# zhang-tao-whu/DVIS_Plus

Measured on AMD Instinct MI355X. Metric: frames/sec DVIS++ R50 offline, 720p T=30 synthetic, higher is better.
Workload: dtype f32 (storage, accumulation, results; the segmenter's dense layers - R50 convolutions from 128 channels on, pixel-decoder projections and FPN output convolution, the deformable encoder's projections and FFN, the decoder's key / value projections - multiply each fp32 operand as two f16 terms on the f1

## Files before the change

dvis_plus_amd/csrc/conv1x1_x3.hip:

```cpp
#include "dvis_common.h"
#include "x3_common.h"

DVIS_EXPORT int64_t dvis_conv_x3_image_bytes(int64_t N, int C, int H, int W);

namespace {

constexpr unsigned kOOB = 0x80000000u;

struct CxArgs {
  const float *x, *bias, *res;
  const void *wp;
  float *y;
  int N, C, K, relu, npass;
  int stride, W_in, OW, H_in;
  int taps;
  long long HW, HW_in, pixels;
  long long tiles;
  float xscale, inv;
  int *flag;
  int tag;
  const float *x2;
  int C2, stride2, W2_in;
  long long HW2_in;
  void *img;
  int XG;
  float oscale;
  int OH;
  const void *ximg;
  int XG_in;
};

__device__ __forceinline__ bool cx_item(const CxArgs &a, long long w, long long *tile, int *pass) {
  const int xcd = blockIdx.x & 7, i = blockIdx.x >> 3, per = gridDim.x >> 3;
  const long long m = i + (long long)per * w;
  const long long u = m / a.npass;
  *pass = (int)(m - u * a.npass);
  *tile = xcd + 8 * u;
  return *tile < a.tiles;
}

struct CxGeom {
  unsigned base;
  int iy, ix;
  int row0;
};
__device__ __forceinline__ CxGeom cx_geom(const CxArgs &a, long long p) {
  CxGeom gm = {kOOB, 0, 0, 0};
  if (p >= a.pixels) return gm;
  const long long n = p / a.HW;
  const int pix = (int)(p - n * a.HW);
  const int oy = pix / a.OW, ox = pix - oy * a.OW, pad = a.taps == 9 ? 1 : 0;
  gm.base = (unsigned)(n * a.C * a.HW_in * 4);
  gm.iy = oy * a.stride - pad, gm.ix = ox * a.stride - pad;
  gm.row0 = (int)(n * a.H_in);
  return gm;
}
__device__ __forceinline__ unsigned cx_tap_offset(const CxArgs &a, const CxGeom &gm, int tap) {
  const int dy = a.taps == 9 ? tap / 3 : 0, dx = a.taps == 9 ? tap - 3 * dy : 0;
  const int iy = gm.iy + dy, ix = gm.ix + dx;
  const bool ok = gm.base != kOOB && iy >= 0 && iy < a.H_in && ix >= 0 && ix < a.W_in;
  return ok ? gm.base + (unsigned)((iy * a.W_in + ix) * 4) : kOOB;
}

__device__ __forceinline__ unsigned cx_tap_offset_img(const CxArgs &a, const CxGeom &gm, int tap, int g) {
  const int dy = a.taps == 9 ? tap / 3 : 0, dx = a.taps == 9 ? tap - 3 * dy : 0;
  const int iy = gm.iy + dy, ix = gm.ix + dx;
  const bool ok = gm.base != kOOB && iy >= 0 && iy < a.H_in && ix >= 0 && ix < a.W_in;
  return ok ? (unsigned)(((gm.row0 + iy) * a.XG_in + (ix >> 5)) * ((a.C / 64) * 8192) + g * 512 + (ix & 31) * 16) : kOOB;
}

__device__ __forceinline__ unsigned cx_geom2(const CxArgs &a, long long p) {
  if (a.C2 == 0 || p >= a.pixels) return kOOB;
  const long long n = p / a.HW;
  const int pix = (int)(p - n * a.HW);
  const int oy = pix / a.OW, ox = pix - oy * a.OW;
  return (unsigned)(n * a.C2 * a.HW2_in * 4) + (unsigned)((oy * a.stride2 * a.W2_in + ox * a.stride2) * 4);
}

template <int NB, int NW, int IK, bool IMGIN = false, bool IMGOUT = false>
__global__ __launch_bounds__(NW * 64) void conv1x1_x3_kernel(const CxArgs a) {
  constexpr int kTile = NW * 32, PW = 2 * IK * NB / NW, STAGES = IK == 4 ? 2 : 3, IPC = 4 / IK;
  static_assert(2 * IK * NB % NW == 0, "the item's pieces must divide among the waves");
  extern __shared__ __attribute__((aligned(1024))) char lds[];
  const int wave = threadIdx.x >> 6, lane = threadIdx.x & 63, j = lane & 31, g = lane >> 5;
  const int NCC = a.C / 64, NC1 = a.taps * NCC, NC = NC1 + a.C2 / 64, NI = IPC * NC;
  long long wcount = 0;
  {
    long long t;
    int q;
    while (cx_item(a, wcount, &t, &q)) ++wcount;
  }
  if (wcount == 0) return;
  const __amdgpu_buffer_rsrc_t rx = dvis_make_rsrc_uniform(a.x, (unsigned)((long long)a.N * a.C * a.HW_in * 4));
  const __amdgpu_buffer_rsrc_t ry = dvis_make_rsrc_uniform(a.y, (unsigned)((long long)a.N * a.K * a.HW * 4));
  const __amdgpu_buffer_rsrc_t rr = dvis_make_rsrc_uniform(a.res ? a.res : a.y, (unsigned)((long long)a.N * a.K * a.HW * 4));
  const unsigned chan = (unsigned)(a.HW_in * 4);
  const __amdgpu_buffer_rsrc_t rx2 = dvis_make_rsrc_uniform(a.C2 ? a.x2 : a.x, a.C2 ? (unsigned)((long long)a.N * a.C2 * a.HW2_in * 4) : 0u);
  const unsigned chan2 = (unsigned)(a.HW2_in * 4);

  typedef Ring<PW, IMGIN ? 8 : 32, NW, STAGES> RingT;
  RingT ring;
  long long iw = 0;
  int ic = 0, ipass;
  {
    long long t;
    cx_item(a, 0, &t, &ipass);
  }
  auto next_offset = [&]() -> size_t {
    const size_t o = ((size_t)ipass * NI + ic) * RingT::kItemBytes;
    if (++ic == NI) {
      ic = 0;
      long long t;
      if (!cx_item(a, ++iw, &t, &ipass)) ipass = 0;
    }
    return o;
  };
  ring.init(a.wp, lds, 1, (int)(wcount * NI), wave, lane);
#pragma unroll
  for (int i = 0; i < RingT::kAhead; ++i)
    if (ring.total > i) ring.issue_at(next_offset());

  float raw[32];
  auto load_raw = [&](unsigned pixoff, int cc, bool second = false) {
    const __amdgpu_buffer_rsrc_t r = second ? rx2 : rx;
    const unsigned ch = second ? chan2 : chan;
    const unsigned vo = pixoff + (unsigned)(8 * g) * ch;
    const unsigned so = (unsigned)(64 * cc) * ch;
#pragma unroll
    for (int s = 0; s < 4; ++s)
#pragma unroll
      for (int e = 0; e < 8; ++e)
        raw[8 * s + e] = __builtin_bit_cast(float, __builtin_amdgcn_raw_buffer_load_b32(r, vo, so + (unsigned)(16 * s + e) * ch, 0));
  };
  const __amdgpu_buffer_rsrc_t rxi = dvis_make_rsrc_uniform(IMGIN ? a.ximg : (const void *)a.x,
                                                            IMGIN ? (unsigned)((long long)a.N * a.H_in * a.XG_in * (a.C / 64) * 8192) : 0u);
  h8 nh[4], nl[4];
  auto load_img = [&](unsigned off, int cc) {
#pragma unroll
    for (int s = 0; s < 4; ++s) {
      nh[s] = __builtin_bit_cast(h8, __builtin_amdgcn_raw_buffer_load_b128(rxi, off, (unsigned)(8192 * cc + 2048 * s), 0));
      nl[s] = __builtin_bit_cast(h8, __builtin_amdgcn_raw_buffer_load_b128(rxi, off, (unsigned)(8192 * cc + 2048 * s + 1024), 0));
    }
  };
  long long tile;
  int pass;
  cx_item(a, 0, &tile, &pass);
  CxGeom gm = cx_geom(a, tile * kTile + wave * 32 + j);
  unsigned gm2 = cx_geom2(a, tile * kTile + wave * 32 + j);
  if constexpr (IMGIN)
    load_img(cx_tap_offset_img(a, gm, 0, g), 0);
  else
    load_raw(cx_tap_offset(a, gm, 0), 0);
  for (long long w = 0; w < wcount; ++w) {
    const long long p = tile * kTile + wave * 32 + j;
    long long ntile = tile;
    int npass_ = pass;
    const bool more = cx_item(a, w + 1, &ntile, &npass_);
    const CxGeom ngm = more ? cx_geom(a, ntile * kTile + wave * 32 + j) : CxGeom{kOOB, 0, 0, 0};
    const unsigned ngm2 = more ? cx_geom2(a, ntile * kTile + wave * 32 + j) : kOOB;
    int tap = 0, cc = 0;
    f16v acc[NB];
#pragma unroll
    for (int nb = 0; nb < NB; ++nb)
#pragma unroll
      for (int i = 0; i < 16; ++i) acc[nb][i] = 0.f;
    const long long n = p / a.HW;
    const unsigned obase = p < a.pixels ? (unsigned)((n * a.K * a.HW + (p - n * a.HW)) * 4) : kOOB;
    const unsigned ochan = (unsigned)(a.HW * 4);
    const int co0 = pass * 32 * NB;
    for (int kc = 0; kc < NC; ++kc) {
      h8 xh[4], xl[4];
      if constexpr (IMGIN) {
#pragma unroll
        for (int s = 0; s < 4; ++s) {
          asm volatile("" : "+v"(nh[s]), "+v"(nl[s]));
          xh[s] = nh[s], xl[s] = nl[s];
        }
        if (++cc == NCC) cc = 0, ++tap;
        const bool first = kc + 1 < NC1;
        load_img(first ? cx_tap_offset_img(a, gm, tap, g) : cx_tap_offset_img(a, ngm, 0, g), first ? cc : 0);
      } else {
#pragma unroll
        for (int i = 0; i < 32; ++i) asm volatile("" : "+v"(raw[i]));
#pragma unroll
        for (int s = 0; s < 4; ++s) {
          const f4 lo4 = {raw[8 * s], raw[8 * s + 1], raw[8 * s + 2], raw[8 * s + 3]};
          const f4 hi4 = {raw[8 * s + 4], raw[8 * s + 5], raw[8 * s + 6], raw[8 * s + 7]};
          split8(lo4, hi4, a.xscale, xh[s], xl[s]);
        }
        if (++cc == NCC) cc = 0, ++tap;
        const bool first = kc + 1 < NC1, sec = !first && kc + 1 < NC;
        const unsigned po = first ? cx_tap_offset(a, gm, tap) : (sec ? gm2 : cx_tap_offset(a, ngm, 0));
        load_raw(po, first ? cc : (sec ? kc + 1 - NC1 : 0), sec);
      }
#pragma unroll
      for (int part = 0; part < IPC; ++part) {
        const char *stage = ring.wait(false);
        ring.begin(ring.more() ? next_offset() : 0);
        mma_item<IK, NB, PW>(stage, lane, acc, xh + IK * part, xl + IK * part, [&](int i) { ring.piece(i); });
      }
    }
    float chk = 0.f;
    if constexpr (NB == 2 || IMGOUT) {
      if (a.img != nullptr) {
        const unsigned gs = (unsigned)(a.K / 64) * 8192u;
        const __amdgpu_buffer_rsrc_t ri = dvis_make_rsrc_uniform(a.img, (unsigned)((long long)a.N * a.OH * a.XG * gs));
        const __amdgpu_buffer_rsrc_t rb = dvis_make_rsrc_uniform(a.bias ? (const void *)a.bias : (const void *)a.img, a.bias ? (unsigned)a.K * 4u : 0u);
        unsigned ibase = kOOB;
        if (p < a.pixels) {
          const int pix = (int)(p - n * a.HW), oy = pix / a.OW, ox = pix - oy * a.OW;
          ibase = (unsigned)(((n * a.OH + oy) * a.XG + (ox >> 5)) * gs + (co0 / 64) * 8192 + g * 512 + (ox & 31) * 16);
        }
#pragma unroll
        for (int nb = 0; nb < NB; ++nb) {
          float v[16];
#pragma unroll
          for (int q = 0; q < 4; ++q) {
            const f4 b = __builtin_bit_cast(f4, __builtin_amdgcn_raw_buffer_load_b128(rb, (unsigned)(co0 + 32 * nb + 8 * q + 4 * g) * 4u, 0, 0));
#pragma unroll
            for (int i = 0; i < 4; ++i) {
              const float t = acc[nb][4 * q + i] * a.inv + b[i];
              chk = __builtin_fmaf(t, 0.f, chk);
              v[4 * q + i] = a.relu ? x3_relu(t) : t;
            }
          }
          h8 hi[2], lo[2];
#pragma unroll
          for (int u = 0; u < 2; ++u) {
            const f4 p0 = {v[8 * u], v[8 * u + 1], v[8 * u + 2], v[8 * u + 3]}, p1 = {v[8 * u + 4], v[8 * u + 5], v[8 * u + 6], v[8 * u + 7]};
            split8(p0, p1, a.oscale, hi[u], lo[u]);
          }
          const h8 ls = lo[0] + lo[1];
          chk = __builtin_fmaf((float)((ls[0] + ls[1]) + (ls[2] + ls[3]) + (ls[4] + ls[5]) + (ls[6] + ls[7])), 0.f, chk);
          store_fragments4(ri, ibase, hi[0], 4096 * nb, lo[0], 4096 * nb + 1024, hi[1], 4096 * nb + 2048, lo[1], 4096 * nb + 3072);
        }
        if (a.flag != nullptr && chk != chk && p < a.pixels) atomicCAS(a.flag, 0, a.tag);
        tile = ntile, pass = npass_, gm = ngm, gm2 = ngm2;
        continue;
      }
    }
#pragma unroll
    for (int nb = 0; nb < NB; ++nb) {
      float rv[16];
#pragma unroll
      for (int r = 0; r < 16; ++r)
        rv[r] = a.res ? __builtin_bit_cast(float, __builtin_amdgcn_raw_buffer_load_b32(
                                                      rr, obase + (unsigned)(co0 + 32 * nb + 8 * (r >> 2) + 4 * g + (r & 3)) * ochan, 0, 0))
                      : 0.f;
#pragma unroll
      for (int q = 0; q < 4; ++q) {
        const int co = co0 + 32 * nb + 8 * q + 4 * g;
        f4 b = {0.f, 0.f, 0.f, 0.f};
        if (a.bias) b = *(const f4 *)(a.bias + co);
#pragma unroll
        for (int i = 0; i < 4; ++i) {
          const unsigned o = obase + (unsigned)(co + i) * ochan;
          float v = acc[nb][4 * q + i] * a.inv + b[i] + rv[4 * q + i];
          chk = __builtin_fmaf(v, 0.f, chk);
          if (a.relu) v = x3_relu(v);
          __builtin_amdgcn_raw_buffer_store_b32(__builtin_bit_cast(unsigned, v), ry, o, 0, 0);
        }
      }
    }
    if (a.flag != nullptr && chk != chk && p < a.pixels) atomicCAS(a.flag, 0, a.tag);
    tile = ntile, pass = npass_, gm = ngm, gm2 = ngm2;
  }
}

__global__ __launch_bounds__(256) void upsample_add_image_kernel(const float *__restrict__ lateral, const float *__restrict__ top,
                                                                 void *__restrict__ img, int N, int C, int H, int W, int h, int w,
                                                                 const float *__restrict__ lat_scale, const float *__restrict__ lat_shift,
                                                                 float oscale) {
  const int NCC = C / 64, XG = (W + 31) / 32;
  const int cc = blockIdx.x, xg = blockIdx.y;
  const int x = threadIdx.x & 31, g = (threadIdx.x >> 5) & 1, S = threadIdx.x >> 6;
  const int px = 32 * xg + x;
  const float sy = (float)h / (float)H, sx = (float)w / (float)W;
  const int pxc = px < W ? px : W - 1;
  float fx = sx * ((float)pxc + 0.5f) - 0.5f;
  fx = fx < 0.f ? 0.f : fx;
  const int x0 = min((int)fx, w - 1), x1 = x0 + (x0 < w - 1 ? 1 : 0);
  const float lx1 = fx - (float)x0, lx0 = 1.f - lx1;
  const __amdgpu_buffer_rsrc_t ri = dvis_make_rsrc_uniform(img, (unsigned)((long long)N * H * XG * NCC * 8192));
  const unsigned rows = (unsigned)N * (unsigned)H;
  for (unsigned row = blockIdx.z * 16u; row < blockIdx.z * 16u + 16u && row < rows; ++row) {
    const unsigned n = row / (unsigned)H;
    const int y = (int)(row - n * (unsigned)H);
    float fy = sy * ((float)y + 0.5f) - 0.5f;
    fy = fy < 0.f ? 0.f : fy;
    const int y0 = min((int)fy, h - 1), y1 = y0 + (y0 < h - 1 ? 1 : 0);
    const float ly1 = fy - (float)y0, ly0 = 1.f - ly1;
    float v[8];
#pragma unroll
    for (int e = 0; e < 8; ++e) {
      const int c = 64 * cc + 32 * (S >> 1) + 16 * (S & 1) + 8 * (e >> 2) + 4 * g + (e & 3);
      const unsigned pl = n * (unsigned)C + (unsigned)c;
      const float *t0 = top + ((size_t)pl * h + y0) * (size_t)w, *t1 = top + ((size_t)pl * h + y1) * (size_t)w;
      float lat = lateral[((size_t)pl * H + y) * (size_t)W + pxc];
      if (lat_scale) lat = lat * lat_scale[pl] + lat_shift[pl];
      v[e] = lat + (ly0 * (lx0 * t0[x0] + lx1 * t0[x1]) + ly1 * (lx0 * t1[x0] + lx1 * t1[x1]));
    }
    const f4 p0 = {v[0], v[1], v[2], v[3]}, p1 = {v[4], v[5], v[6], v[7]};
    h8 hi, lo;
    split8(p0, p1, oscale, hi, lo);
    const unsigned G = row * (unsigned)XG + (unsigned)xg;
    const unsigned off = (G * (unsigned)NCC + (unsigned)cc) * 8192u + (unsigned)(S * 2048 + g * 512 + x * 16);
    store_fragments2(ri, off, hi, 0, lo, 1024);
  }
}

}

DVIS_EXPORT int dvis_upsample_add_image(const float *lateral, const float *lat_scale, const float *lat_shift, const float *top, void *image,
                                        int N, int C, int H, int W, int h, int w, int oexp, void *stream) {
  DVIS_REQUIRE(lateral && top && image, "dvis_upsample_add_image: null pointer");
  DVIS_REQUIRE((lat_scale == nullptr) == (lat_shift == nullptr), "dvis_upsample_add_image: scale and shift together");
  DVIS_REQUIRE(N > 0 && C > 0 && C % 64 == 0 && H > 0 && W > 0 && h > 0 && w > 0, "dvis_upsample_add_image: bad sizes");
  DVIS_REQUIRE((uintptr_t)image % 16 == 0 && dvis_conv_x3_image_bytes(N, C, H, W) < ((int64_t)1 << 31), "dvis_upsample_add_image: a 16-byte "
               "aligned image below 2 GiB");
  const int per = 16 * 65535 / H;
  DVIS_REQUIRE(per >= 1 && (W + 31) / 32 <= 65535, "dvis_upsample_add_image: map too large (%d x %d)", H, W);
  for (int i = 0; i < N; i += per) {
    const int n = N - i < per ? N - i : per;
    hipLaunchKernelGGL(upsample_add_image_kernel, dim3(C / 64, (W + 31) / 32, (n * H + 15) / 16), dim3(256), 0, (hipStream_t)stream,
                       lateral + (size_t)i * C * H * W, top + (size_t)i * C * h * w,
                       (char *)image + (size_t)i * H * ((W + 31) / 32) * (C / 64) * 8192, n, C, H, W, h, w,
                       lat_scale ? lat_scale + (size_t)i * C : nullptr, lat_shift ? lat_shift + (size_t)i * C : nullptr, ldexpf(1.f, oexp));
  }
  return dvis_check_launch("dvis_upsample_add_image");
}

DVIS_EXPORT int dvis_conv1x1_x3_supported(int C, int K, int64_t N, int64_t HW_in, int64_t HW_out) {
  if (C < 64 || C % 64 != 0 || C > 4096) return 0;
  if (!(K == 64 || K == 128 || (K > 0 && K % 256 == 0 && K <= 8192))) return 0;
  if (N <= 0 || HW_out <= 0 || HW_in < HW_out) return 0;
  if (N * C * HW_in * 4 >= ((int64_t)1 << 31) || N * K * HW_out * 4 >= ((int64_t)1 << 31)) return 0;
  return 1;
}

DVIS_EXPORT int64_t dvis_conv1x1_x3_packed_bytes(int C, int K) {
  if (!dvis_conv1x1_x3_supported(C, K, 1, 1, 1)) return -1;
  return (int64_t)(C / 16) * (K / 32) * 2 * kPiece;
}

DVIS_EXPORT int dvis_conv1x1_x3_pack(const float *w, int K, int C, int wexp, void *packed, void *stream) {
  DVIS_REQUIRE(w && packed, "dvis_conv1x1_x3_pack: null operand");
  DVIS_REQUIRE(dvis_conv1x1_x3_supported(C, K, 1, 1, 1), "dvis_conv1x1_x3_pack: (C, K) = (%d, %d) is not served", C, K);
  DVIS_REQUIRE(wexp >= -60 && wexp <= 60, "dvis_conv1x1_x3_pack: wexp = %d", wexp);
  const int NB = K == 64 ? 2 : K == 128 ? 4 : 8;
  const int64_t fragments = (int64_t)(C / 16) * (K / 32) * 64;
  hipLaunchKernelGGL(x3_pack_kernel, dim3((unsigned)((fragments + 255) / 256)), dim3(256), 0, (hipStream_t)stream, w, (int64_t)C, K, C,
                     NB, 0, ldexpf(1.f, wexp), (_Float16 *)packed, fragments);
  return dvis_check_launch("dvis_conv1x1_x3_pack");
}

static int cx_launch(const float *x, const void *packed, const float *bias, const float *res, float *y, int N, int C, int K, int H, int W,
                     int stride, int taps, int xexp, int wexp, int relu, void *stream, const float *x2 = nullptr, int C2 = 0, int H2 = 0,
                     int W2 = 0, int stride2 = 1, void *image = nullptr, int oexp = 0, const void *ximg = nullptr);

DVIS_EXPORT int dvis_conv1x1_x3_dual(const float *x, const float *x2, const void *packed, const float *bias, const float *res, float *y,
                                     int N, int C, int C2, int K, int H, int W, int H2, int W2, int stride2, int xexp, int wexp, int relu,
                                     void *stream) {
  DVIS_REQUIRE(x2 != nullptr && C2 >= 64 && C2 % 64 == 0 && C2 <= 4096, "dvis_conv1x1_x3_dual: C2 %% 64 == 0 (got %d)", C2);
  DVIS_REQUIRE((stride2 == 1 || stride2 == 2) && (H2 + stride2 - 1) / stride2 == H && (W2 + stride2 - 1) / stride2 == W,
               "dvis_conv1x1_x3_dual: x2 (%d x %d, stride %d) must down-sample onto x's %d x %d map", H2, W2, stride2, H, W);
  DVIS_REQUIRE((long long)N * C2 * H2 * W2 * 4 < ((long long)1 << 31) && (uintptr_t)x2 % 16 == 0, "dvis_conv1x1_x3_dual: x2 below 2 GiB, 16-byte aligned");
  return cx_launch(x, packed, bias, res, y, N, C, K, H, W, 1, 1, xexp, wexp, relu, stream, x2, C2, H2, W2, stride2);
}

DVIS_EXPORT int dvis_conv1x1_x3(const float *x, const void *packed, const float *bias, const float *res, float *y, int N, int C, int K,
                                int H, int W, int stride, int xexp, int wexp, int relu, void *stream) {
  return cx_launch(x, packed, bias, res, y, N, C, K, H, W, stride, 1, xexp, wexp, relu, stream);
}

DVIS_EXPORT int dvis_conv1x1_x3_image(const float *x, const void *packed, const float *bias, void *image, int N, int C, int H, int W, int xexp,
                                      int wexp, int oexp, int relu, void *stream) {
  DVIS_REQUIRE(image != nullptr && (uintptr_t)image % 16 == 0, "dvis_conv1x1_x3_image: null / unaligned image");
  DVIS_REQUIRE((long long)N * H * ((W + 31) / 32) * 8192 < ((long long)1 << 31), "dvis_conv1x1_x3_image: the image must stay below 2 GiB");
  return cx_launch(x, packed, bias, nullptr, nullptr, N, C, 64, H, W, 1, 1, xexp, wexp, relu, stream, nullptr, 0, 0, 0, 1, image, oexp);
}

DVIS_EXPORT int64_t dvis_conv_x3_image_bytes(int64_t N, int C, int H, int W) {
  if (N < 0 || C <= 0 || C % 64 != 0 || H <= 0 || W <= 0) return -1;
  return N * H * ((W + 31) / 32) * (int64_t)(C / 64) * 8192;
}

DVIS_EXPORT int dvis_conv_x3_pack_image(const float *w, int K, int C, int taps, int wexp, void *packed, void *stream) {
  DVIS_REQUIRE(w && packed, "dvis_conv_x3_pack_image: null operand");
  DVIS_REQUIRE(taps == 1 || taps == 9, "dvis_conv_x3_pack_image: taps = %d", taps);
  DVIS_REQUIRE(dvis_conv1x1_x3_supported(C, K, 1, 1, 1) && K >= 128, "dvis_conv_x3_pack_image: (C, K) = (%d, %d) is not served", C, K);
  DVIS_REQUIRE(wexp >= -60 && wexp <= 60, "dvis_conv_x3_pack_image: wexp = %d", wexp);
  const int NB = K == 128 ? 4 : 8;
  const int64_t fragments = (int64_t)(taps * C / 16) * (K / 32) * 64;
  hipLaunchKernelGGL(x3_pack_kernel, dim3((unsigned)((fragments + 255) / 256)), dim3(256), 0, (hipStream_t)stream, w, (int64_t)taps * C, K,
                     taps * C, NB, 1, ldexpf(1.f, wexp), (_Float16 *)packed, fragments, taps);
  return dvis_check_launch("dvis_conv_x3_pack_image");
}

DVIS_EXPORT int dvis_conv_x3_image(const void *ximg, const float *x, const void *packed, const float *bias, const float *res, float *y,
                                   void *image, int N, int C, int K, int H, int W, int stride, int taps, int xexp, int wexp, int oexp, int relu,
                                   void *stream) {
  DVIS_REQUIRE(ximg != nullptr || image != nullptr, "dvis_conv_x3_image: neither side is an operand image (use dvis_conv1x1_x3 / dvis_conv3x3_x3)");
  DVIS_REQUIRE((ximg != nullptr) != (x != nullptr), "dvis_conv_x3_image: exactly one of ximg and x");
  DVIS_REQUIRE((image != nullptr) != (y != nullptr), "dvis_conv_x3_image: exactly one of image and y");
  DVIS_REQUIRE(K == 128 || K % 256 == 0, "dvis_conv_x3_image: K = %d (128 or a multiple of 256)", K);
  DVIS_REQUIRE(taps == 1 || taps == 9, "dvis_conv_x3_image: taps = %d", taps);
  DVIS_REQUIRE(image == nullptr || res == nullptr, "dvis_conv_x3_image: an image output takes no residual");
  DVIS_REQUIRE(((uintptr_t)ximg | (uintptr_t)image) % 16 == 0, "dvis_conv_x3_image: images must be 16-byte aligned");
  const int OH = (H + stride - 1) / stride, OW = (W + stride - 1) / stride;
  DVIS_REQUIRE(dvis_conv_x3_image_bytes(N, C, H, W) < ((int64_t)1 << 31) && dvis_conv_x3_image_bytes(N, K, OH, OW) < ((int64_t)1 << 31),
               "dvis_conv_x3_image: images must stay below 2 GiB");
  return cx_launch(x, packed, bias, res, y, N, C, K, H, W, stride, taps, xexp, wexp, relu, stream, nullptr, 0, 0, 0, 1, image, oexp, ximg);
}

DVIS_EXPORT int64_t dvis_conv3x3_x3_packed_bytes(int C, int K) {
  const int64_t b = dvis_conv1x1_x3_packed_bytes(C, K);
  return b < 0 ? b : 9 * b;
}

DVIS_EXPORT int dvis_conv3x3_x3_pack(const float *w, int K, int C, int wexp, void *packed, void *stream) {
  DVIS_REQUIRE(w && packed, "dvis_conv3x3_x3_pack: null operand");
  DVIS_REQUIRE(dvis_conv1x1_x3_supported(C, K, 1, 1, 1), "dvis_conv3x3_x3_pack: (C, K) = (%d, %d) is not served", C, K);
  DVIS_REQUIRE(wexp >= -60 && wexp <= 60, "dvis_conv3x3_x3_pack: wexp = %d", wexp);
  const int NB = K == 64 ? 2 : K == 128 ? 4 : 8;
  const int64_t fragments = (int64_t)(9 * C / 16) * (K / 32) * 64;
  hipLaunchKernelGGL(x3_pack_kernel, dim3((unsigned)((fragments + 255) / 256)), dim3(256), 0, (hipStream_t)stream, w, (int64_t)9 * C, K, 9 * C,
                     NB, 0, ldexpf(1.f, wexp), (_Float16 *)packed, fragments, 9);
  return dvis_check_launch("dvis_conv3x3_x3_pack");
}

DVIS_EXPORT int dvis_conv3x3_x3(const float *x, const void *packed, const float *bias, const float *res, float *y, int N, int C, int K,
                                int H, int W, int stride, int xexp, int wexp, int relu, void *stream) {
  return cx_launch(x, packed, bias, res, y, N, C, K, H, W, stride, 9, xexp, wexp, relu, stream);
}

static int cx_launch(const float *x, const void *packed, const float *bias, const float *res, float *y, int N, int C, int K, int H, int W,
                     int stride, int taps, int xexp, int wexp, int relu, void *stream, const float *x2, int C2, int H2, int W2, int stride2,
                     void *image, int oexp, const void *ximg) {
  DVIS_REQUIRE((x || ximg) && packed && (y || image), "dvis_conv1x1_x3: null operand");
  DVIS_REQUIRE(stride == 1 || stride == 2, "dvis_conv1x1_x3: stride %d", stride);
  const int OH = (H + stride - 1) / stride, OW = (W + stride - 1) / stride;
  DVIS_REQUIRE(dvis_conv1x1_x3_supported(C, K, N, (int64_t)H * W, (int64_t)OH * OW), "dvis_conv1x1_x3: shape (N %d, C %d, K %d, %d x %d, "
               "stride %d) is not served (C %% 64 == 0, K = 64 / 128 or K %% 256 == 0, tensors below 2 GiB)", N, C, K, H, W, stride);
  DVIS_REQUIRE((uintptr_t)x % 16 == 0 && (uintptr_t)y % 16 == 0 && (uintptr_t)packed % 16 == 0 && (bias == nullptr || (uintptr_t)bias % 16 == 0),
               "dvis_conv1x1_x3: operands must be 16-byte aligned");
  CxArgs a = {};
  a.x = x, a.bias = bias, a.res = res, a.wp = packed, a.y = y, a.N = N, a.C = C, a.K = K, a.relu = relu;
  a.stride = stride, a.W_in = W, a.H_in = H, a.taps = taps, a.OW = OW, a.HW = (long long)OH * OW, a.HW_in = (long long)H * W;
  a.pixels = a.HW * N;
  a.xscale = ldexpf(1.f, xexp), a.inv = ldexpf(1.f, -(xexp + wexp));
  const X3Guard gd = dvis_x3_guard();
  a.flag = gd.flag, a.tag = gd.tag;
  a.x2 = x2, a.C2 = x2 ? C2 : 0, a.stride2 = stride2, a.W2_in = W2, a.HW2_in = (long long)H2 * W2;
  a.img = image, a.XG = (OW + 31) / 32, a.oscale = ldexpf(1.f, oexp), a.OH = OH;
  a.ximg = ximg, a.XG_in = (W + 31) / 32;
  const int grid = dvis_x3_persistent_cus();
  hipStream_t st = (hipStream_t)stream;
  static const int nw = getenv("DVIS_X3_CONV_WAVES") ? atoi(getenv("DVIS_X3_CONV_WAVES")) : 8;
  a.npass = K <= 128 ? 1 : K / 256;
#define DVIS_CX_LAUNCH(NBV, NWV, IKV)                                                                              \
  {                                                                                                                \
    static DvisLdsOptIn opted;                                                                                     \
    typedef Ring<2 * IKV * NBV / NWV, 32, NWV, (IKV == 4 ? 2 : 3)> R;                                              \
    a.tiles = (a.pixels + 32 * NWV - 1) / (32 * NWV);                                                              \
    const size_t lds = (IKV == 4 ? 2 : 3) * R::kItemBytes;                                                         \
    const int rc = dvis_lds_opt_in((const void *)conv1x1_x3_kernel<NBV, NWV, IKV>, lds, &opted, "dvis_conv1x1_x3"); \
    if (rc != DVIS_OK) return rc;                                                                                  \
    hipLaunchKernelGGL((conv1x1_x3_kernel<NBV, NWV, IKV>), dim3(grid), dim3(NWV * 64), lds, st, a);                \
  }
#define DVIS_CX_LAUNCH_IMG(NBV, IKV, INV, OUTV)                                                                                    \
  {                                                                                                                                \
    static DvisLdsOptIn opted;                                                                                                     \
    typedef Ring<2 * IKV * NBV / 8, 8, 8, (IKV == 4 ? 2 : 3)> R;                                                                   \
    a.tiles = (a.pixels + 255) / 256;                                                                                              \
    const size_t lds = (IKV == 4 ? 2 : 3) * R::kItemBytes;                                                                         \
    const int rc = dvis_lds_opt_in((const void *)conv1x1_x3_kernel<NBV, 8, IKV, INV, OUTV>, lds, &opted, "dvis_conv_x3_image");    \
    if (rc != DVIS_OK) return rc;                                                                                                  \
    hipLaunchKernelGGL((conv1x1_x3_kernel<NBV, 8, IKV, INV, OUTV>), dim3(grid), dim3(512), lds, st, a);                            \
    return dvis_check_launch("dvis_conv_x3_image");                                                                                \
  }
  if (ximg != nullptr || (image != nullptr && K != 64)) {
    DVIS_REQUIRE(x2 == nullptr, "dvis_conv_x3_image: no second source");
    if (K == 128) {
      if (ximg && image) DVIS_CX_LAUNCH_IMG(4, 2, true, true)
      if (ximg) DVIS_CX_LAUNCH_IMG(4, 2, true, false)
      DVIS_CX_LAUNCH_IMG(4, 2, false, true)
    }
    if (ximg && image) DVIS_CX_LAUNCH_IMG(8, 4, true, true)
    if (ximg) DVIS_CX_LAUNCH_IMG(8, 4, true, false)
    DVIS_CX_LAUNCH_IMG(8, 4, false, true)
  }
#undef DVIS_CX_LAUNCH_IMG
  static const int ik = getenv("DVIS_X3_CONV_ITEM") ? atoi(getenv("DVIS_X3_CONV_ITEM")) : 4;
  if (K == 64) {
    if (nw == 8) DVIS_CX_LAUNCH(2, 8, 2) else DVIS_CX_LAUNCH(2, 4, 2)
  } else if (K == 128) {
    if (nw == 8) DVIS_CX_LAUNCH(4, 8, 2) else DVIS_CX_LAUNCH(4, 4, 2)
  } else if (ik == 4) {
    DVIS_CX_LAUNCH(8, 8, 4)
  } else {
    if (nw == 8) DVIS_CX_LAUNCH(8, 8, 2) else DVIS_CX_LAUNCH(8, 4, 2)
  }
#undef DVIS_CX_LAUNCH
  return dvis_check_launch("dvis_conv1x1_x3");
}
```

dvis_plus_amd/csrc/fused_elementwise.hip:

```cpp
#include <math.h>

#include "dvis_common.h"

namespace {

template <int V>
__global__ __launch_bounds__(256) void add_layernorm_kernel(const float *__restrict__ x, const float *__restrict__ res,
                                                            int64_t res_row_stride, const float *__restrict__ gamma,
                                                            const float *__restrict__ beta, float *__restrict__ out,
                                                            size_t rows, int C, float eps,
                                                            const float *__restrict__ pos, size_t pos_rows,
                                                            float *__restrict__ out_pos) {
  const int lane = threadIdx.x & 63;
  const size_t row = (size_t)blockIdx.x * 4 + (threadIdx.x >> 6);
  if (row >= rows) return;
  const float4 *xr = reinterpret_cast<const float4 *>(x + row * C);
  const float4 *rr = res ? reinterpret_cast<const float4 *>(res + row * res_row_stride) : nullptr;
  float4 v[V];
  float sum = 0.f;
#pragma unroll
  for (int i = 0; i < V; ++i) {
    const int c4 = lane + 64 * i;
    if (c4 * 4 < C) {
      v[i] = xr[c4];
// ... 481 lines not shown

DVIS_EXPORT int dvis_add_layernorm(const float *x, const float *res, int64_t res_row_stride, const float *gamma,
                                   const float *beta, float *out, int64_t rows, int C, float eps, void *stream) {
  return add_layernorm_launch(x, res, res_row_stride, gamma, beta, out, rows, C, eps, nullptr, 0, nullptr, stream);
}

DVIS_EXPORT int dvis_add_layernorm_pos(const float *x, const float *res, int64_t res_row_stride, const float *gamma,
                                       const float *beta, float *out, const float *pos, int64_t pos_rows, float *out_pos,
                                       int64_t rows, int C, float eps, void *stream) {
  DVIS_REQUIRE(pos && out_pos, "add_layernorm_pos: null pos / out_pos");
  return add_layernorm_launch(x, res, res_row_stride, gamma, beta, out, rows, C, eps, pos, pos_rows, out_pos, stream);
}

static int upsample_add_launch(const float *lateral, const float *top, float *out, int64_t planes, int H, int W, int h,
                               int w, const float *lat_scale, const float *lat_shift, void *stream) {
  DVIS_REQUIRE(planes >= 0 && H > 0 && W > 0 && h > 0 && w > 0, "upsample_add: bad sizes");
  if (planes == 0) return DVIS_OK;
  DVIS_REQUIRE(lateral && top && out, "upsample_add: null pointer");
  DVIS_REQUIRE((lat_scale == nullptr) == (lat_shift == nullptr), "upsample_add: scale and shift come together");
  DVIS_REQUIRE(planes < (1ll << 31), "upsample_add: too many planes");
  if (W % 4 != 0 || (((uintptr_t)lateral | (uintptr_t)out) & 15) != 0) {
    const long long tot = (long long)planes * H * W;
    long long nb = (tot + 255) / 256;
    if (nb > 256 * 32) nb = 256 * 32;
    hipLaunchKernelGGL(upsample_add_scalar_kernel, dim3((unsigned)nb), dim3(256), 0, (hipStream_t)stream, lateral, top, out, tot, H, W,
                       h, w, lat_scale, lat_shift);
    return dvis_check_launch("upsample_add_scalar_kernel");
  }
  const size_t total = (size_t)planes * H * (W / 4);
  size_t blocks = (total + 255) / 256;
  if (blocks > 256 * 32) blocks = 256 * 32;
  DVIS_REQUIRE(total < (1ull << 32), "upsample_add: more than 2^32 output quads");
  const bool x2 = H == 2 * h && W == 2 * w && (w & 1) == 0 && ((uintptr_t)top & 7) == 0;
  if (x2)
    hipLaunchKernelGGL(upsample_add_kernel<true>, dim3((unsigned)blocks), dim3(256), 0, (hipStream_t)stream, lateral, top,
                       out, (int)planes, H, W, h, w, lat_scale, lat_shift);
  else
    hipLaunchKernelGGL(upsample_add_kernel<false>, dim3((unsigned)blocks), dim3(256), 0, (hipStream_t)stream, lateral, top,
                       out, (int)planes, H, W, h, w, lat_scale, lat_shift);
  return dvis_check_launch("upsample_add_kernel");
}

DVIS_EXPORT int dvis_dwconv3x3_tokens(const float *x, float *out, int64_t batch_stride, int B, int h, int w, int C, const float *weight,
                                      const float *bias, int gelu, void *stream) {
  DVIS_REQUIRE(x && out && weight, "dwconv3x3_tokens: null pointer");
  DVIS_REQUIRE(B >= 0 && h > 0 && w > 0 && C > 0 && C % 4 == 0 && batch_stride % 4 == 0 && batch_stride >= (int64_t)h * w * C,
               "dwconv3x3_tokens: C %% 4 == 0 and a batch stride that is a multiple of 4 floats >= h * w * C are required");
  DVIS_REQUIRE(((uintptr_t)x | (uintptr_t)out | (uintptr_t)(bias ? bias : weight)) % 16 == 0, "dwconv3x3_tokens: 16-byte alignment");
  DVIS_REQUIRE(x != out, "dwconv3x3_tokens: in place is not possible (neighbouring tokens are read)");
  if (B == 0) return DVIS_OK;
  const int64_t strips = (int64_t)h * ((w + 3) / 4);
  DVIS_REQUIRE(strips * B < ((int64_t)1 << 32), "dwconv3x3_tokens: too many tokens");
  hipLaunchKernelGGL(dwconv3x3_tokens_kernel, dim3((unsigned)((strips * B + 3) / 4), (C / 4 + 63) / 64), dim3(256), 0, (hipStream_t)stream, x,
                     out, batch_stride, B, h, w, C, weight, bias, gelu);
  return dvis_check_launch("dwconv3x3_tokens_kernel");
}

DVIS_EXPORT int dvis_adapter_res2(const float *g, const float *c1, const float *x1, const float *scale, const float *shift, float *out,
                                  int B, int C, int h8, int w8, void *stream) {
  DVIS_REQUIRE(g && c1 && scale && shift && out, "adapter_res2: null pointer");
  DVIS_REQUIRE(((uintptr_t)g | (uintptr_t)c1 | (uintptr_t)out) % 16 == 0, "adapter_res2: g / c1 / out must be 16-byte aligned");
  DVIS_REQUIRE(B >= 0 && C > 0 && C % 64 == 0 && h8 > 0 && w8 > 0 && h8 % 2 == 0 && w8 % 2 == 0,
               "adapter_res2: C %% 64 == 0 and an even stride-8 grid are required (C %d, grid %d x %d)", C, h8, w8);
  DVIS_REQUIRE((int64_t)B * h8 <= 65535 && C / 64 <= 65535, "adapter_res2: grid too large (B * rows %lld)", (long long)B * h8);
  if (B == 0) return DVIS_OK;
  hipLaunchKernelGGL(adapter_res2_kernel, dim3((w8 + 31) / 32, C / 64, B * h8), dim3(256), 0, (hipStream_t)stream, g, c1, x1, scale, shift,
                     out, C, h8, w8);
  return dvis_check_launch("adapter_res2_kernel");
}

DVIS_EXPORT int dvis_upsample_add(const float *lateral, const float *top, float *out, int64_t planes, int H, int W, int h,
                                  int w, void *stream) {
  return upsample_add_launch(lateral, top, out, planes, H, W, h, w, nullptr, nullptr, stream);
}

DVIS_EXPORT int dvis_upsample_add_affine(const float *lateral, const float *lat_scale, const float *lat_shift,
                                         const float *top, float *out, int64_t planes, int H, int W, int h, int w,
                                         void *stream) {
  DVIS_REQUIRE(lat_scale && lat_shift, "upsample_add_affine: null scale / shift");
  return upsample_add_launch(lateral, top, out, planes, H, W, h, w, lat_scale, lat_shift, stream);
}

DVIS_EXPORT int dvis_bias_relu_maxpool(const float *x, const float *bias, float *out, int64_t planes, int C, int H, int W,
                                       void *stream) {
  DVIS_REQUIRE(planes >= 0 && C > 0 && H > 0 && W > 0, "bias_relu_maxpool: bad sizes");
  if (planes == 0) return DVIS_OK;
  DVIS_REQUIRE(x && out, "bias_relu_maxpool: null pointer");
  DVIS_REQUIRE(H % 2 == 0 && W % 8 == 0 && (((uintptr_t)x | (uintptr_t)out) & 15) == 0,
               "bias_relu_maxpool: needs even H, W %% 8 == 0 and 16-byte aligned x / out (H=%d W=%d)", H, W);
  const size_t total = (size_t)planes * (H / 2) * (W / 8);
  DVIS_REQUIRE(planes < (1ll << 31) && total < (1ull << 32), "bias_relu_maxpool: too many planes / outputs");
  size_t blocks = (total + 255) / 256;
  if (blocks > 256 * 32) blocks = 256 * 32;
  hipLaunchKernelGGL(bias_relu_maxpool_kernel, dim3((unsigned)blocks), dim3(256), 0, (hipStream_t)stream, x, bias, out,
                     (int)planes, C, H, W);
  return dvis_check_launch("bias_relu_maxpool_kernel");
}

namespace {

__global__ __launch_bounds__(1024) void group_norm_affine_kernel(const float *__restrict__ x, const float *__restrict__ gamma,
                                                                 const float *__restrict__ beta, float *__restrict__ scale,
                                                                 float *__restrict__ shift, int C, int G, long long HW,
                                                                 float eps, int vec) {
  __shared__ double s_sum[16], s_sq[16];
  const int Cg = C / G;
  const int n = blockIdx.x / G, g = blockIdx.x - n * G;
  const long long count = (long long)Cg * HW, count4 = count / 4;
  const float4 *xp = reinterpret_cast<const float4 *>(x + ((size_t)n * C + (size_t)g * Cg) * HW);
  double sum = 0.0, sq = 0.0;
  if (vec) {
    for (long long i = threadIdx.x; i < count4; i += 1024) {
      const float4 v = xp[i];
      sum += ((double)v.x + (double)v.y) + ((double)v.z + (double)v.w);
      sq += ((double)v.x * v.x + (double)v.y * v.y) + ((double)v.z * v.z + (double)v.w * v.w);
    }
  } else {
    const float *xs = reinterpret_cast<const float *>(xp);
    for (long long i = threadIdx.x; i < count; i += 1024) {
      const double v = (double)xs[i];
      sum += v;
      sq += v * v;
    }
  }
#pragma unroll
  for (int o = 32; o > 0; o >>= 1) {
    sum += __shfl_down(sum, o);
    sq += __shfl_down(sq, o);
  }
  const int wv = threadIdx.x >> 6;
  if ((threadIdx.x & 63) == 0) {
    s_sum[wv] = sum;
    s_sq[wv] = sq;
  }
  __syncthreads();
  if (threadIdx.x < Cg) {
    double ts = 0.0, tq = 0.0;
#pragma unroll
    for (int i = 0; i < 16; ++i) {
      ts += s_sum[i];
      tq += s_sq[i];
    }
    const double mean = ts / (double)count;
    double var = tq / (double)count - mean * mean;
    var = var < 0.0 ? 0.0 : var;
    const float rstd = (float)(1.0 / sqrt(var + (double)eps));
    const int c = g * Cg + threadIdx.x;
    const float a = rstd * (gamma ? gamma[c] : 1.f);
    scale[(size_t)n * C + c] = a;
    shift[(size_t)n * C + c] = (beta ? beta[c] : 0.f) - (float)mean * a;
  }
}

__global__ __launch_bounds__(256) void scale_shift_act_kernel(float *__restrict__ x, const float *__restrict__ scale,
                                                              const float *__restrict__ shift, int HW4, int chunks, int relu) {
  const unsigned plane = blockIdx.x / chunks;
  const int chunk = blockIdx.x - plane * chunks;
  const float a = scale[plane], b = shift[plane];
  float4 *xp = reinterpret_cast<float4 *>(x) + (size_t)plane * HW4;
  for (int i = chunk * 256 + threadIdx.x; i < HW4; i += chunks * 256) {
    float4 v = xp[i];
    v.x = v.x * a + b; v.y = v.y * a + b; v.z = v.z * a + b; v.w = v.w * a + b;
    if (relu) {
      v.x = fmaxf(v.x, 0.f); v.y = fmaxf(v.y, 0.f); v.z = fmaxf(v.z, 0.f); v.w = fmaxf(v.w, 0.f);
    }
    xp[i] = v;
  }
}

__global__ __launch_bounds__(256) void scale_shift_act_scalar_kernel(float *__restrict__ x, const float *__restrict__ scale,
                                                                     const float *__restrict__ shift, long long HW, long long total,
                                                                     int relu) {
  for (long long i = (long long)blockIdx.x * 256 + threadIdx.x; i < total; i += (long long)gridDim.x * 256) {
    const long long plane = i / HW;
    const float v = x[i] * scale[plane] + shift[plane];
    x[i] = relu ? fmaxf(v, 0.f) : v;
  }
}

}

DVIS_EXPORT int dvis_group_norm_affine(const float *x, const float *gamma, const float *beta, float *scale, float *shift,
                                       int64_t N, int C, int G, int64_t HW, float eps, void *stream) {
  DVIS_REQUIRE(N >= 0 && C > 0 && G > 0 && HW > 0 && C % G == 0, "group_norm_affine: bad sizes (C=%d G=%d)", C, G);
  if (N == 0) return DVIS_OK;
  DVIS_REQUIRE(x && scale && shift, "group_norm_affine: null pointer");
  DVIS_REQUIRE(C / G <= 1024, "group_norm_affine: at most 1024 channels per group");
  const int vec = ((int64_t)(C / G) * HW) % 4 == 0 && ((uintptr_t)x & 15) == 0;
  DVIS_REQUIRE(N * G < (1ll << 31), "group_norm_affine: too many groups");
  hipLaunchKernelGGL(group_norm_affine_kernel, dim3((unsigned)(N * G)), dim3(1024), 0, (hipStream_t)stream, x, gamma, beta,
                     scale, shift, C, G, (long long)HW, eps, vec);
  return dvis_check_launch("group_norm_affine_kernel");
}

DVIS_EXPORT int dvis_scale_shift_act(float *x, const float *scale, const float *shift, int64_t planes, int64_t HW, int relu,
                                     void *stream) {
  DVIS_REQUIRE(planes >= 0 && HW > 0, "scale_shift_act: bad sizes");
  if (planes == 0) return DVIS_OK;
  DVIS_REQUIRE(x && scale && shift, "scale_shift_act: null pointer");
  if (HW % 4 != 0 || ((uintptr_t)x & 15) != 0) {
    const long long total = (long long)planes * HW;
    const long long blocks = (total + 255) / 256;
    hipLaunchKernelGGL(scale_shift_act_scalar_kernel, dim3((unsigned)(blocks > 65535 * 16 ? 65535 * 16 : blocks)), dim3(256), 0,
                       (hipStream_t)stream, x, scale, shift, (long long)HW, total, relu);
    return dvis_check_launch("scale_shift_act_scalar_kernel");
  }
  const int HW4 = (int)(HW / 4);
  int chunks = (HW4 + 1023) / 1024;
  if (chunks < 1) chunks = 1;
  DVIS_REQUIRE(planes * chunks < (1ll << 31), "scale_shift_act: too many planes");
  hipLaunchKernelGGL(scale_shift_act_kernel, dim3((unsigned)(planes * chunks)), dim3(256), 0, (hipStream_t)stream, x, scale,
                     shift, HW4, chunks, relu);
  return dvis_check_launch("scale_shift_act_kernel");
}
```

dvis_plus_amd/functions.py:

```python
import collections
import ctypes
import math
import os
import threading

import torch
from torch.autograd import Function
from torch.autograd.function import once_differentiable

from . import cpu_ops, derived, native
from .cpu_ops import ms_deform_attn_core_pytorch


def _torch_path(op, x, why):
    if os.environ.get("DVIS_STRICT", "1") != "0" and x.is_cuda and not torch.is_grad_enabled():
        raise RuntimeError(f"DVIS_STRICT: {op} would run its torch formulation on a GPU tensor ({why}; shape "
                           f"{tuple(x.shape)}, dtype {x.dtype}, contiguous {x.is_contiguous()})")


class no_autocast:

    def __enter__(self):
        import contextlib
        self._stack = contextlib.ExitStack()
# ... 524 lines not shown
        dq, dk, dv = attention_backward(q, k, v, grad_out, ctx.nheads)
        need = ctx.needs_input_grad
        return dq if need[0] else None, dk if need[1] else None, dv if need[2] else None, None, None


def vps_argmax(mask_logits_kthw, scores, first_resize_size, img_size, out_hw):
    K, T, h, w = mask_logits_kthw.shape
    m = mask_logits_kthw
    if not m.is_cuda or m.dtype != torch.float32 or m.stride(3) != 1 or m.stride(2) != w:
        raise RuntimeError("vps_argmax: logits must be a float32 GPU (K, T, h, w) view with contiguous (h, w) maps")
    scores = scores.to(torch.float32).contiguous()
    oh, ow = int(out_hw[0]), int(out_hw[1])
    ids = torch.empty((T, oh, ow), dtype=torch.int32, device=m.device)
    conf = torch.empty((T, oh, ow), dtype=torch.uint8, device=m.device)
    areas = torch.empty((3, K), dtype=torch.int32, device=m.device)
    with torch.cuda.device(m.device):
        rc = native.lib().dvis_vps_argmax(
            ctypes.c_void_p(m.data_ptr()), m.stride(0), m.stride(1), native.dev_ptr(scores, "scores"), K, T, h, w,
            int(first_resize_size[0]), int(first_resize_size[1]), int(img_size[0]), int(img_size[1]), oh, ow,
            native.dev_ptr(ids, "ids"), native.dev_ptr(conf, "conf"), native.dev_ptr(areas, "areas"),
            native.stream_ptr(m.device))
    native.check(rc, "dvis_vps_argmax")
    return ids, conf.bool(), areas


def resize2_gt0(mask_logits_kthw, first_resize_size, img_size, out_hw):
    K, T, h, w = mask_logits_kthw.shape
    m = mask_logits_kthw
    if not m.is_cuda or m.dtype != torch.float32 or m.stride(3) != 1 or m.stride(2) != w:
        raise RuntimeError("resize2_gt0: logits must be a float32 GPU (K, T, h, w) view with contiguous (h, w) maps")
    oh, ow = int(out_hw[0]), int(out_hw[1])
    out = torch.empty((K, T, oh, ow), dtype=torch.uint8, device=m.device)
    with torch.cuda.device(m.device):
        rc = native.lib().dvis_resize2_gt0(
            ctypes.c_void_p(m.data_ptr()), m.stride(0), m.stride(1), K, T, h, w, int(first_resize_size[0]),
            int(first_resize_size[1]), int(img_size[0]), int(img_size[1]), oh, ow, native.dev_ptr(out, "out"),
            native.stream_ptr(m.device))
    native.check(rc, "dvis_resize2_gt0")
    return out.view(torch.bool)


def resize2(mask_logits_kthw, first_resize_size, img_size, out_hw, sigmoid=False):
    K, T, h, w = mask_logits_kthw.shape
    m = mask_logits_kthw
    if not m.is_cuda or m.dtype != torch.float32 or m.stride(3) != 1 or m.stride(2) != w:
        raise RuntimeError("resize2: logits must be a float32 GPU (K, T, h, w) view with contiguous (h, w) maps")
    oh, ow = int(out_hw[0]), int(out_hw[1])
    out = torch.empty((K, T, oh, ow), dtype=torch.float32, device=m.device)
    with torch.cuda.device(m.device):
        rc = native.lib().dvis_resize2(
            ctypes.c_void_p(m.data_ptr()), m.stride(0), m.stride(1), K, T, h, w, int(first_resize_size[0]),
            int(first_resize_size[1]), int(img_size[0]), int(img_size[1]), oh, ow, 1 if sigmoid else 0,
            native.dev_ptr(out, "out"), native.stream_ptr(m.device))
    native.check(rc, "dvis_resize2")
    return out


def vss_argmax(mask_logits_qthw, mask_cls, first_resize_size, img_size, out_hw):
    Q, T, h, w = mask_logits_qthw.shape
    m = mask_logits_qthw
    if not m.is_cuda or m.dtype != torch.float32 or m.stride(3) != 1 or m.stride(2) != w:
        raise RuntimeError("vss_argmax: logits must be a float32 GPU (Q, T, h, w) view with contiguous (h, w) maps")
    C = mask_cls.shape[1]
    Cp = (C + 31) // 32 * 32
    cls = torch.nn.functional.pad(mask_cls.to(torch.float32), (0, Cp - C)).contiguous()
    oh, ow = int(out_hw[0]), int(out_hw[1])
    out = torch.empty((T, oh, ow), dtype=torch.int64, device=m.device)
    with torch.cuda.device(m.device):
        rc = native.lib().dvis_vss_argmax(
            ctypes.c_void_p(m.data_ptr()), m.stride(0), m.stride(1), native.dev_ptr(cls, "mask_cls"), Cp, Q, C, T,
            h, w, int(first_resize_size[0]), int(first_resize_size[1]), int(img_size[0]), int(img_size[1]), oh, ow,
            native.dev_ptr(out, "out"), native.stream_ptr(m.device))
    native.check(rc, "dvis_vss_argmax")
    return out


def add_layer_norm(x, res, norm, pos=None):
    C = x.shape[-1]

    def with_pos(out):
        return out if pos is None else (out, out + pos.reshape(1, -1, C))
    if not (x.is_cuda and x.dtype == torch.float32 and x.is_contiguous() and C % 4 == 0 and C <= 1024
            and norm.weight is not None and not torch.is_grad_enabled()):
        _torch_path("add_layer_norm", x, "needs contiguous fp32 rows with C % 4 == 0, C <= 1024 and an affine norm")
        return with_pos(norm(x if res is None else x + res))
    rp, rs = None, 0
    if res is not None:
        if res.shape != x.shape or res.dtype != torch.float32 or not res.is_cuda:
            _torch_path("add_layer_norm", x, "residual must be fp32 of x's shape")
            return with_pos(norm(x + res))
        if not res.is_contiguous():
            res = res.contiguous()
        rp, rs = ctypes.c_void_p(res.data_ptr()), C
    out = torch.empty_like(x)
    rows = x.numel() // C
    with torch.cuda.device(x.device):
        if pos is None:
            rc = native.lib().dvis_add_layernorm(ctypes.c_void_p(x.data_ptr()), rp, rs, native.dev_ptr(norm.weight, "gamma"),
                                                 native.dev_ptr(norm.bias, "beta"), ctypes.c_void_p(out.data_ptr()),
                                                 rows, C, float(norm.eps), native.stream_ptr(x.device))
        else:
            pos_rows = pos.numel() // C
            if x.dim() != 3 or x.shape[1] != pos_rows or pos.dtype != torch.float32 or not pos.is_cuda:
                raise RuntimeError("add_layer_norm: pos must be a float32 GPU (S, C) embedding for x of shape (N, S, C)")
            pos = pos.contiguous()
            out_pos = torch.empty_like(x)
            rc = native.lib().dvis_add_layernorm_pos(
                ctypes.c_void_p(x.data_ptr()), rp, rs, native.dev_ptr(norm.weight, "gamma"),
                native.dev_ptr(norm.bias, "beta"), ctypes.c_void_p(out.data_ptr()), native.dev_ptr(pos, "pos"), pos_rows,
                ctypes.c_void_p(out_pos.data_ptr()), rows, C, float(norm.eps), native.stream_ptr(x.device))
    native.check(rc, "dvis_add_layernorm")
    return out if pos is None else (out, out_pos)


def bias_relu_maxpool(x, bias=None):
    N, C, H, W = x.shape
    if not (x.is_cuda and x.dtype == torch.float32 and x.is_contiguous() and H % 2 == 0 and W % 8 == 0
            and not torch.is_grad_enabled()):
        _torch_path("bias_relu_maxpool", x, "needs contiguous fp32 NCHW with H % 2 == 0 and W % 8 == 0")
        import torch.nn.functional as F
        if bias is not None:
            x = x + bias.view(1, -1, 1, 1)
        return F.max_pool2d(torch.relu(x), kernel_size=3, stride=2, padding=1)
    out = torch.empty((N, C, H // 2, W // 2), dtype=torch.float32, device=x.device)
    with torch.cuda.device(x.device):
        rc = native.lib().dvis_bias_relu_maxpool(native.dev_ptr(x, "x"),
                                                 None if bias is None else native.dev_ptr(bias, "bias"),
                                                 native.dev_ptr(out, "out"), N * C, C, H, W, native.stream_ptr(x.device))
    native.check(rc, "dvis_bias_relu_maxpool")
    return out


def _fused_map_ok(x):
    return x.is_cuda and x.dtype == torch.float32 and x.is_contiguous() and not torch.is_grad_enabled()


def group_norm_affine(x, norm):
    N, C, H, W = x.shape
    G = norm.num_groups
    if not (_fused_map_ok(x) and C // G <= 1024):
        _torch_path("group_norm_affine", x, "needs contiguous fp32 NCHW, at most 1024 channels per group")
        return None
    scale = torch.empty(N * C, dtype=torch.float32, device=x.device)
    shift = torch.empty(N * C, dtype=torch.float32, device=x.device)
    with torch.cuda.device(x.device):
        rc = native.lib().dvis_group_norm_affine(
            native.dev_ptr(x, "x"), None if norm.weight is None else native.dev_ptr(norm.weight.detach(), "gamma"),
            None if norm.bias is None else native.dev_ptr(norm.bias.detach(), "beta"), native.dev_ptr(scale, "scale"),
            native.dev_ptr(shift, "shift"), N, C, G, H * W, float(norm.eps), native.stream_ptr(x.device))
    native.check(rc, "dvis_group_norm_affine")
    return scale, shift


def scale_shift_act_(x, scale, shift, relu=False):
    N, C, H, W = x.shape
    with torch.cuda.device(x.device):
        rc = native.lib().dvis_scale_shift_act(native.dev_ptr(x, "x"), native.dev_ptr(scale, "scale"),
                                               native.dev_ptr(shift, "shift"), N * C, H * W, 1 if relu else 0,
                                               native.stream_ptr(x.device))
    native.check(rc, "dvis_scale_shift_act")
    return x


def upsample_add(lateral, top, lat_affine=None):
    N, C, H, W = lateral.shape
    if not (_fused_map_ok(lateral) and top.dtype == torch.float32):
        _torch_path("upsample_add", lateral, "needs contiguous fp32 NCHW")
        import torch.nn.functional as F
        if lat_affine is not None:
            lateral = lateral * lat_affine[0].view(N, C, 1, 1) + lat_affine[1].view(N, C, 1, 1)
        return lateral + F.interpolate(top, size=(H, W), mode="bilinear", align_corners=False)
    top = top.contiguous()
    out = torch.empty_like(lateral)
    with torch.cuda.device(lateral.device):
        if lat_affine is None:
            rc = native.lib().dvis_upsample_add(native.dev_ptr(lateral, "lateral"), native.dev_ptr(top, "top"),
                                                native.dev_ptr(out, "out"), N * C, H, W, top.shape[-2], top.shape[-1],
                                                native.stream_ptr(lateral.device))
        else:
            rc = native.lib().dvis_upsample_add_affine(
                native.dev_ptr(lateral, "lateral"), native.dev_ptr(lat_affine[0], "scale"),
                native.dev_ptr(lat_affine[1], "shift"), native.dev_ptr(top, "top"), native.dev_ptr(out, "out"), N * C, H,
                W, top.shape[-2], top.shape[-1], native.stream_ptr(lateral.device))
    native.check(rc, "dvis_upsample_add")
    return out


def dwconv3x3_tokens(x, level_shapes, weight, bias, gelu=False):
    B, N, C = x.shape
    if not (x.is_cuda and x.dtype == torch.float32 and x.is_contiguous() and weight.dtype == torch.float32 and C % 4 == 0
            and sum(h * w for h, w in level_shapes) == N and weight.shape == (C, 1, 3, 3)):
        raise RuntimeError(f"dwconv3x3_tokens: needs a contiguous float32 GPU (B, N, C) tensor, C % 4 == 0, levels summing to N "
                           f"(x {tuple(x.shape)}, levels {list(level_shapes)})")
    out = torch.empty_like(x)
    wt = weight.detach().reshape(C, 9).contiguous()
    bptr = None if bias is None else native.dev_ptr(bias.detach().contiguous(), "bias")
    off = 0
    with torch.cuda.device(x.device):
        for h, w in level_shapes:
            rc = native.lib().dvis_dwconv3x3_tokens(ctypes.c_void_p(x.data_ptr() + 4 * off * C), ctypes.c_void_p(out.data_ptr() + 4 * off * C),
                                                    N * C, B, h, w, C, native.dev_ptr(wt, "weight"), bptr, int(gelu),
                                                    native.stream_ptr(x.device))
            native.check(rc, "dvis_dwconv3x3_tokens")
            off += h * w
    return out


def adapter_res2(g, c1, x1_tokens, scale, shift, h8, w8):
    B, C = c1.shape[0], c1.shape[1]
    for t, name in ((g, "g"), (c1, "c1"), (scale, "scale"), (shift, "shift")) + (((x1_tokens, "x1"),) if x1_tokens is not None else ()):
        if not (t.is_cuda and t.dtype == torch.float32 and t.is_contiguous()):
            raise RuntimeError(f"adapter_res2: {name} must be a contiguous float32 GPU tensor")
    if g.shape != (B * h8 * w8, 4 * C) or c1.shape != (B, C, 2 * h8, 2 * w8) or \
            (x1_tokens is not None and x1_tokens.shape != (B, (h8 // 2) * (w8 // 2), C)):
        raise RuntimeError(f"adapter_res2: shapes g {tuple(g.shape)}, c1 {tuple(c1.shape)}, x1 "
                           f"{None if x1_tokens is None else tuple(x1_tokens.shape)} do not match a {h8} x {w8} stride-8 grid")
    out = torch.empty_like(c1)
    with torch.cuda.device(c1.device):
        rc = native.lib().dvis_adapter_res2(native.dev_ptr(g, "g"), native.dev_ptr(c1, "c1"),
                                            None if x1_tokens is None else native.dev_ptr(x1_tokens, "x1"),
                                            native.dev_ptr(scale, "scale"), native.dev_ptr(shift, "shift"), native.dev_ptr(out, "out"),
                                            B, C, h8, w8, native.stream_ptr(c1.device))
    native.check(rc, "dvis_adapter_res2")
    return out


OWN_GEMM_DEFAULT = os.environ.get("DVIS_DETERMINISTIC", "1") != "0"


class gemm_sizes_as:
    _tls = threading.local()

    def __init__(self, rows=None, batch=None):
        self.rows, self.batch = rows, batch

    @staticmethod
    def current():
        return getattr(gemm_sizes_as._tls, "pin", (None, None))

    def __enter__(self):
        self.prev = gemm_sizes_as.current()
        gemm_sizes_as._tls.pin = (self.rows, self.batch)

    def __exit__(self, *exc):
        gemm_sizes_as._tls.pin = self.prev


def _gemm_config(M, N, K, batch, config):
    rows, b = gemm_sizes_as.current()
    if config >= 0 or (rows is None and b is None):
        return config
    return native.lib().dvis_gemm_pick_config(rows or M, N, K, b or batch)


def _rows2d(x, K):
    if x.dim() == 2 and x.stride(1) == 1 and x.stride(0) >= K:
        return x, x.stride(0)
    if not x.is_contiguous():
        x = x.contiguous()
    return x.view(-1, K), K


def gemm_nt(a, w, bias=None, relu=False, res=None, config=-1, head_major=0, out=None):
    K = a.shape[-1]
    N = w.shape[0]
    if not (a.is_cuda and a.dtype == torch.float32 and w.dtype == torch.float32 and w.dim() == 2 and w.shape[1] == K
            and w.stride(1) == 1):
        raise RuntimeError("gemm_nt: needs float32 GPU operands a (..., K), w (N, K) with unit inner strides")
    a2, lda = _rows2d(a, K)
    M = a2.shape[0]
    if head_major:
        if N % head_major or head_major % 4 or res is not None:
            raise RuntimeError("gemm_nt: head_major needs N % d == 0, d % 4 == 0 and no residual")
        out = torch.empty((N // head_major, M, head_major), dtype=torch.float32, device=a.device)
    elif out is None:
        out = torch.empty((*a.shape[:-1], N), dtype=torch.float32, device=a.device)
    elif not (out.is_cuda and out.dtype == torch.float32 and out.is_contiguous() and out.numel() == M * N):
        raise RuntimeError("gemm_nt: out must be a contiguous float32 GPU tensor of M * N elements")
    rp, ldres = None, 0
    if res is not None:
        if res.numel() != out.numel() or res.shape[-1] != N or res.dtype != torch.float32 or not res.is_cuda:
            raise RuntimeError("gemm_nt: res must be a float32 GPU tensor of the output's shape")
        r2, ldres = _rows2d(res, N)
        rp = ctypes.c_void_p(r2.data_ptr())
    bp = None
    if bias is not None:
        if bias.dtype != torch.float32 or bias.numel() != N or not bias.is_contiguous():
            raise RuntimeError("gemm_nt: bias must be a contiguous float32 (N,) tensor")
        bp = ctypes.c_void_p(bias.data_ptr())
    with torch.cuda.device(a.device):
        rc = native.lib().dvis_gemm_nt_hm(ctypes.c_void_p(a2.data_ptr()), lda, 0, ctypes.c_void_p(w.data_ptr()), w.stride(0), 0,
                                          bp, rp, ldres, 0, ctypes.c_void_p(out.data_ptr()), head_major or N, 0, M, N, K, 1,
                                          1 if relu else 0, _gemm_config(M, N, K, 1, config), int(head_major),
                                          M * head_major, native.stream_ptr(a.device))
    native.check(rc, "dvis_gemm_nt")
    return out


def gemm_nt_stacked(a, w, bias=None, config=-1):
    L, N, K = w.shape
    if not (a.is_cuda and a.dtype == torch.float32 and w.dtype == torch.float32 and a.dim() == 2 and a.stride(1) == 1
            and a.shape[1] == L * K and w.is_contiguous()):
        raise RuntimeError("gemm_nt_stacked: needs float32 GPU operands a (M, L * K) with unit inner stride, contiguous w (L, N, K)")
    if bias is not None and not (bias.dtype == torch.float32 and bias.shape == (L, N) and bias.is_contiguous()):
        raise RuntimeError("gemm_nt_stacked: bias must be a contiguous float32 (L, N) tensor")
    M = a.shape[0]
# ... 583 lines not shown

def x3_ffn_ok(x, lin1, lin2):
    K, H, N = lin1.weight.shape[1], lin1.weight.shape[0], lin2.weight.shape[0]
    return (x.is_cuda and x.dtype == torch.float32 and not torch.is_grad_enabled() and x.shape[-1] == K
            and lin2.weight.shape[1] == H and lin1.bias is not None and lin2.bias is not None
            and native.lib().dvis_x3_ffn_packed_bytes(K, H, N) > 0)


def x3_ffn_ln(x, lin1, lin2, norm, pos=None, xexp=None, hexp=None):
    w1, w2 = lin1.weight, lin2.weight
    H, K = w1.shape
    N = w2.shape[0]
    x2, ldx = _x3_rows(x, "x")

    def make():
        a, b = w1.detach().contiguous(), w2.detach().contiguous()
        e1, e2 = _x3_wexp(a), _x3_wexp(b)
        buf = torch.empty(native.lib().dvis_x3_ffn_packed_bytes(K, H, N), dtype=torch.uint8, device=a.device)
        with torch.cuda.device(a.device):
            native.check(native.lib().dvis_x3_ffn_pack(ctypes.c_void_p(a.data_ptr()), K, ctypes.c_void_p(b.data_ptr()), H, K, H,
                                                       N, e1, e2, ctypes.c_void_p(buf.data_ptr()),
                                                       native.stream_ptr(a.device)), "dvis_x3_ffn_pack")
        return buf, e1, e2
    buf, e1, e2 = _x3_cache(w1, [w1, w2], make, kind="ffn")
    out = torch.empty((*x.shape[:-1], N), dtype=torch.float32, device=x.device)
    pos, pos_rows, out2 = _x3_pos(pos, x, N)
    with torch.cuda.device(x.device):
        native.check(native.lib().dvis_x3_ffn_ln(
            ctypes.c_void_p(x2.data_ptr()), ldx, x2.shape[0], K, H, N, ctypes.c_void_p(buf.data_ptr()),
            X3_XEXP if xexp is None else xexp, e1, X3_XEXP if hexp is None else hexp, e2,
            native.dev_ptr(lin1.bias.detach(), "b1"), native.dev_ptr(lin2.bias.detach(), "b2"),
            native.dev_ptr(norm.weight.detach(), "gamma"), native.dev_ptr(norm.bias.detach(), "beta"), float(norm.eps),
            None if pos is None else ctypes.c_void_p(pos.data_ptr()), pos_rows, ctypes.c_void_p(out.data_ptr()),
            None if out2 is None else ctypes.c_void_p(out2.data_ptr()), N, native.stream_ptr(x.device)), "dvis_x3_ffn_ln")
    return out if out2 is None else (out, out2)


def maps_to_tokens(maps, affines=None, pos=None):
    affines = affines or [None] * len(maps)
    N, C = maps[0].shape[:2]
    if not all(m.is_cuda and m.dtype == torch.float32 and m.is_contiguous() for m in maps) or torch.is_grad_enabled():
        _torch_path("maps_to_tokens", maps[0], "needs contiguous fp32 NCHW maps")
        maps = [m if a is None else m * a[0].view(N, C, 1, 1) + a[1].view(N, C, 1, 1) for m, a in zip(maps, affines)]
        out = torch.cat([m.flatten(2).transpose(1, 2) for m in maps], 1)
        return out if pos is None else (out, out + pos.reshape(1, -1, C))
    S = sum(m.shape[2] * m.shape[3] for m in maps)
    out = torch.empty((N, S, C), dtype=torch.float32, device=maps[0].device)
    out_pos = pp = None
    if pos is not None:
        if pos.numel() != S * C or pos.dtype != torch.float32 or not pos.is_cuda:
            raise RuntimeError("maps_to_tokens: pos must be a float32 GPU (S, C) embedding")
        pos = pos.contiguous()
        out_pos = torch.empty_like(out)
        pp = native.dev_ptr(pos, "pos")
    row0 = 0
    with torch.cuda.device(out.device):
        for m, a in zip(maps, affines):
            HW = m.shape[2] * m.shape[3]
            rc = native.lib().dvis_nchw_to_tokens_affine(
                ctypes.c_void_p(m.data_ptr()), None if a is None else native.dev_ptr(a[0], "scale"),
                None if a is None else native.dev_ptr(a[1], "shift"), pp, ctypes.c_void_p(out.data_ptr()),
                None if out_pos is None else ctypes.c_void_p(out_pos.data_ptr()), N, C, HW, S, row0,
                native.stream_ptr(out.device))
            native.check(rc, "dvis_nchw_to_tokens_affine")
            row0 += HW
    return out if pos is None else (out, out_pos)


def normalize_pad_ok(x, mean):
    return bool(x.is_cuda and x.dim() == 4 and x.dtype in (torch.uint8, torch.float32) and x.is_contiguous()
                and mean.numel() == x.shape[1] and mean.dtype == torch.float32 and not torch.is_grad_enabled())


def normalize_pad(x, mean, std, Hp, Wp):
    N, C, H, W = x.shape
    out = torch.empty((N, C, Hp, Wp), dtype=torch.float32, device=x.device)
    with torch.cuda.device(x.device):
        native.check(native.lib().dvis_normalize_pad(
            native.dev_ptr(x, "frames"), int(x.dtype == torch.uint8), native.dev_ptr(out, "out"), N * C, C, H, W, Hp, Wp,
            native.dev_ptr(mean.detach().reshape(-1), "pixel_mean"), native.dev_ptr(std.detach().reshape(-1), "pixel_std"),
            native.stream_ptr(x.device)), "dvis_normalize_pad")
    return out


def tokens_to_map(tokens, row0, h, w):
    N, S, C = tokens.shape
    if not (tokens.is_cuda and tokens.dtype == torch.float32 and tokens.is_contiguous() and not torch.is_grad_enabled()):
        return tokens[:, row0:row0 + h * w].transpose(1, 2).reshape(N, C, h, w)
    out = torch.empty((N, C, h, w), dtype=torch.float32, device=tokens.device)
    with torch.cuda.device(tokens.device):
        native.check(native.lib().dvis_tokens_to_nchw(ctypes.c_void_p(tokens.data_ptr()), ctypes.c_void_p(out.data_ptr()), N, C, h * w,
                                                      S, row0, native.stream_ptr(tokens.device)), "dvis_tokens_to_nchw")
    return out


def conv1x1(x, weight, bias=None):
    Co, Ci = weight.shape[:2]
    if conv1x1_x3_ok(x, weight):
        return conv1x1_x3(x, weight, bias)
    if bias is not None and CONV1X1_MFMA and x.is_cuda and x.dim() == 4 and x.is_contiguous() and x.dtype == torch.float32 \
            and weight.dtype == torch.float32 and not torch.is_grad_enabled() \
            and native.lib().dvis_conv1x1_mfma_supported(Ci, Co, x.shape[2] * x.shape[3]):
        return conv1x1_mfma(x, weight, bias)
    if x.is_cuda and Ci >= Co and x.is_contiguous() and x.dim() == 4 and x.dtype == weight.dtype \
            and not torch.is_grad_enabled():
        N, _, H, W = x.shape
        y = torch.bmm(weight.detach().view(1, Co, Ci).expand(N, Co, Ci), x.view(N, Ci, H * W)).view(N, Co, H, W)
        return y if bias is None else bias_act_(y, bias.detach(), None, relu=False)
    return torch.nn.functional.conv2d(x, weight, bias)


def conv1x1_bias_act(x, weight, bias=None, res=None, relu=False):
    Co, Ci = weight.shape[:2]
    if x.is_cuda and x.dim() == 4 and x.dtype == torch.float32 and weight.dtype == torch.float32 and x.is_contiguous() \
            and not torch.is_grad_enabled() and (res is None or (res.is_contiguous() and res.dtype == torch.float32)):
        N, _, H, W = x.shape
        if Ci >= X3_CONV1X1_MIN_CI and conv1x1_x3_ok(x, weight, 1, res):
            return conv1x1_x3(x, weight, bias, res, relu)
        if native.lib().dvis_conv1x1_supported(Ci, Co, H * W) and (res is None or res.shape == (N, Co, H, W)):
            w2 = weight.detach().reshape(Co, Ci)
            if not w2.is_contiguous():
                w2 = w2.contiguous()
            out = torch.empty((N, Co, H, W), dtype=torch.float32, device=x.device)
            with torch.cuda.device(x.device):
                rc = native.lib().dvis_conv1x1_bias_act(
                    native.dev_ptr(x, "x"), native.dev_ptr(w2, "weight"),
                    None if bias is None else native.dev_ptr(bias.detach(), "bias"),
                    None if res is None else native.dev_ptr(res, "res"), native.dev_ptr(out, "out"), N, Ci, Co, H * W,
                    1 if relu else 0, native.stream_ptr(x.device))
            native.check(rc, "dvis_conv1x1_bias_act")
            return out
        if CONV1X1_MFMA and native.lib().dvis_conv1x1_mfma_supported(Ci, Co, H * W) and (res is None or res.shape == (N, Co, H, W)):
            return conv1x1_mfma(x, weight, bias, res, relu)
    return bias_act_(conv1x1(x, weight), None if bias is None else bias.detach(), res, relu)


def conv1x1_x3_ok(x, weight, stride=1, res=None):
    if not (x3_on() and x.is_cuda and x.dim() == 4 and x.dtype == torch.float32 and weight.dtype == torch.float32 and x.is_contiguous()
            and not torch.is_grad_enabled()):
        return False
    N, Ci, H, W = x.shape
    Co = weight.shape[0]
    OH, OW = (H + stride - 1) // stride, (W + stride - 1) // stride
    if res is not None and not (res.is_contiguous() and res.dtype == torch.float32 and tuple(res.shape) == (N, Co, OH, OW)):
        return False
    return N == 0 or bool(native.lib().dvis_conv1x1_x3_supported(Ci, Co, 1, H * W, OH * OW))


def _conv_x3_chunks(N, Ci, Co, HW_in, HW_out):
    per = max(Ci * HW_in, Co * HW_out) * 4
    return max(1, min(N, (2 ** 31 - 1) // per))


def conv1x1_x3(x, weight, bias=None, res=None, relu=False, stride=1, xexp=None):
    N, Ci, H, W = x.shape
    Co = weight.shape[0]

    def make():
        return _x3_pack_conv1x1(weight.detach().reshape(Co, Ci).contiguous())
    buf, wexp = _x3_cache(weight, [weight], make, kind="conv1x1")
    OH, OW = (H + stride - 1) // stride, (W + stride - 1) // stride
    out = torch.empty((N, Co, OH, OW), dtype=torch.float32, device=x.device)
    step = _conv_x3_chunks(N, Ci, Co, H * W, OH * OW)
    with torch.cuda.device(x.device):
        for i in range(0, N, step):
            n = min(step, N - i)
            native.check(native.lib().dvis_conv1x1_x3(
                native.dev_ptr(x[i:i + n], "x"), ctypes.c_void_p(buf.data_ptr()),
                None if bias is None else native.dev_ptr(bias.detach(), "bias"),
                None if res is None else native.dev_ptr(res[i:i + n], "res"), native.dev_ptr(out[i:i + n], "out"), n, Ci, Co, H, W,
                stride, X3_CONV_XEXP if xexp is None else xexp, wexp, 1 if relu else 0, native.stream_ptr(x.device)),
                "dvis_conv1x1_x3")
    return out


X3_DUAL = os.environ.get("DVIS_X3_DUAL", "1") != "0"


def conv1x1_x3_dual_ok(a, w3, x, ws, stride2):
    if not (X3_DUAL and conv1x1_x3_ok(a, w3) and x.is_cuda and x.dim() == 4 and x.dtype == torch.float32 and x.is_contiguous()
            and ws.dtype == torch.float32 and ws.shape[0] == w3.shape[0] and stride2 in (1, 2)):
        return False
    N, C, H, W = a.shape
    N2, C2, H2, W2 = x.shape
    Co = w3.shape[0]
    return (N2 == N and C2 % 64 == 0 and 64 <= C2 <= 4096 and (H2 + stride2 - 1) // stride2 == H and (W2 + stride2 - 1) // stride2 == W
            and (C + C2) <= 4096 and bool(native.lib().dvis_conv1x1_x3_supported(C + C2, Co, 1, H * W, H * W))
            and C2 * H2 * W2 * 4 < 2 ** 31)


def conv1x1_x3_dual(a, w3, b3, x, ws, bs, relu=True, stride2=1, xexp=None):
    N, C, H, W = a.shape
    _, C2, H2, W2 = x.shape
    Co = w3.shape[0]

    def make():
        wcat = torch.cat([w3.detach().reshape(Co, C), ws.detach().reshape(Co, C2)], 1).contiguous()
        buf, e = _x3_pack_conv1x1(wcat)
        bias = None
        if b3 is not None or bs is not None:
            bias = (0 if b3 is None else b3.detach()) + (0 if bs is None else bs.detach())
        return buf, e, bias
    buf, wexp, bias = _x3_cache(w3, [w3, ws, b3, bs], make, kind="conv1x1 + shortcut")
    out = torch.empty((N, Co, H, W), dtype=torch.float32, device=a.device)
    step = min(_conv_x3_chunks(N, C, Co, H * W, H * W), _conv_x3_chunks(N, C2, Co, H2 * W2, H * W))
    with torch.cuda.device(a.device):
        for i in range(0, N, step):
            n = min(step, N - i)
            native.check(native.lib().dvis_conv1x1_x3_dual(
                native.dev_ptr(a[i:i + n], "a"), native.dev_ptr(x[i:i + n], "x"), ctypes.c_void_p(buf.data_ptr()),
                None if bias is None else native.dev_ptr(bias, "bias"), None, native.dev_ptr(out[i:i + n], "out"), n, C, C2, Co, H, W,
                H2, W2, stride2, X3_CONV_XEXP if xexp is None else xexp, wexp, 1 if relu else 0, native.stream_ptr(a.device)),
                "dvis_conv1x1_x3_dual")
    return out


def conv3x3_x3_ok(x, weight, stride=1, res=None):
    return weight.dim() == 4 and tuple(weight.shape[2:]) == (3, 3) and conv1x1_x3_ok(x, weight, stride, res)


def conv3x3_x3(x, weight, bias=None, res=None, relu=False, stride=1, xexp=None):
    N, Ci, H, W = x.shape
    Co = weight.shape[0]

    def make():
        return _x3_pack_conv3x3(weight.detach().contiguous())
    buf, wexp = _x3_cache(weight, [weight], make, kind="conv3x3")
    OH, OW = (H + stride - 1) // stride, (W + stride - 1) // stride
    out = torch.empty((N, Co, OH, OW), dtype=torch.float32, device=x.device)
    step = _conv_x3_chunks(N, Ci, Co, H * W, OH * OW)
    with torch.cuda.device(x.device):
        for i in range(0, N, step):
            n = min(step, N - i)
            native.check(native.lib().dvis_conv3x3_x3(
                native.dev_ptr(x[i:i + n], "x"), ctypes.c_void_p(buf.data_ptr()),
                None if bias is None else native.dev_ptr(bias.detach(), "bias"),
                None if res is None else native.dev_ptr(res[i:i + n], "res"), native.dev_ptr(out[i:i + n], "out"), n, Ci, Co, H, W,
                stride, X3_CONV_XEXP if xexp is None else xexp, wexp, 1 if relu else 0, native.stream_ptr(x.device)),
                "dvis_conv3x3_x3")
    return out


X3_IMAGES = os.environ.get("DVIS_X3_IMAGES", "1") != "0"


class OperandImage:

    def __init__(self, data, N, C, H, W, exp):
        self.data, self.N, self.C, self.H, self.W, self.exp = data, N, C, H, W, exp

    @property
    def device(self):
        return self.data.device

    def images(self, i, n):
        per = self.data.numel() // self.N
        return self.data[i * per:(i + n) * per]


def x3_images_ok(N, C, K, H, W, device, taps=1, stride=1):
    if not (X3_IMAGES and x3_on() and device.type == "cuda" and not torch.is_grad_enabled()):
        return False
    if taps not in (1, 9) or C % 64 != 0 or not (K == 128 or K % 256 == 0) or N <= 0:
        return False
    OH, OW = (H + stride - 1) // stride, (W + stride - 1) // stride
    return bool(native.lib().dvis_conv1x1_x3_supported(C, K, 1, H * W, OH * OW))


def _image_chunks(N, C, K, H, W, OH, OW):
    per = max(C * H * ((W + 31) // 32 * 32), K * OH * ((OW + 31) // 32 * 32)) * 4
    return max(1, min(N, (2 ** 31 - 1) // per))


def upsample_add_image(lateral, top, lat_affine=None, oexp=None):
    N, C, H, W = lateral.shape
    lib = native.lib()
    oe = X3_CONV_XEXP if oexp is None else oexp
    top = top.contiguous()
    data = torch.empty(lib.dvis_conv_x3_image_bytes(N, C, H, W), dtype=torch.uint8, device=lateral.device)
    img = OperandImage(data, N, C, H, W, oe)
    step = _image_chunks(N, C, C, H, W, H, W)
    with torch.cuda.device(lateral.device):
        for i in range(0, N, step):
            n = min(step, N - i)
            sc = None if lat_affine is None else native.dev_ptr(lat_affine[0].reshape(N, C)[i:i + n], "scale")
            sh = None if lat_affine is None else native.dev_ptr(lat_affine[1].reshape(N, C)[i:i + n], "shift")
            native.check(lib.dvis_upsample_add_image(native.dev_ptr(lateral[i:i + n], "lateral"), sc, sh, native.dev_ptr(top[i:i + n], "top"),
                                                     ctypes.c_void_p(img.images(i, n).data_ptr()), n, C, H, W, top.shape[-2], top.shape[-1], oe,
                                                     native.stream_ptr(lateral.device)), "dvis_upsample_add_image")
    return img


def conv_x3_image(src, weight, bias=None, res=None, relu=False, stride=1, out_image=False, oexp=None, xexp=None):
    lib = native.lib()
    from_img = isinstance(src, OperandImage)
    if not (from_img or out_image):
        raise ValueError("conv_x3_image: neither side is an operand image")
    N, C, H, W = (src.N, src.C, src.H, src.W) if from_img else src.shape
    K, taps = weight.shape[0], weight.shape[2] * weight.shape[3]
    dev = weight.device

    def make():
        w2 = weight.detach().contiguous()
        if from_img:
            return _x3_packed(w2, lib.dvis_conv1x1_x3_packed_bytes(C, K) * taps, lambda e, buf, st: lib.dvis_conv_x3_pack_image(
                native.dev_ptr(w2, "weight"), K, C, taps, e, buf, st), "dvis_conv_x3_pack_image")
        return _x3_pack_conv1x1(w2.reshape(K, C)) if taps == 1 else _x3_pack_conv3x3(w2)
    kind = ("conv%dx%d" % ((1, 1) if taps == 1 else (3, 3))) + (" image-in" if from_img else "")
    buf, wexp = _x3_cache(weight, [weight], make, kind=kind)
    OH, OW = (H + stride - 1) // stride, (W + stride - 1) // stride
    xe = src.exp if from_img else (X3_CONV_XEXP if xexp is None else xexp)
    oe = X3_CONV_XEXP if oexp is None else oexp
    if out_image:
        out = OperandImage(torch.empty(lib.dvis_conv_x3_image_bytes(N, K, OH, OW), dtype=torch.uint8, device=dev), N, K, OH, OW, oe)
    else:
        out = torch.empty((N, K, OH, OW), dtype=torch.float32, device=dev)
    step = _image_chunks(N, C, K, H, W, OH, OW)
    with torch.cuda.device(dev):
        for i in range(0, N, step):
            n = min(step, N - i)
            native.check(lib.dvis_conv_x3_image(
                ctypes.c_void_p(src.images(i, n).data_ptr()) if from_img else None, None if from_img else native.dev_ptr(src[i:i + n], "x"),
                ctypes.c_void_p(buf.data_ptr()), None if bias is None else native.dev_ptr(bias.detach(), "bias"),
                None if res is None else native.dev_ptr(res[i:i + n], "res"), None if out_image else native.dev_ptr(out[i:i + n], "out"),
                ctypes.c_void_p(out.images(i, n).data_ptr()) if out_image else None, n, C, K, H, W, stride, taps, xe, wexp, oe, 1 if relu else 0,
                native.stream_ptr(dev)), "dvis_conv_x3_image")
    return out


X3_BNECK = os.environ.get("DVIS_X3_BNECK", "1") != "0"


def bneck_stage_x3_ok(x, blocks):
    if not (X3_BNECK and x3_on() and x.is_cuda and x.dim() == 4 and x.dtype == torch.float32 and x.is_contiguous()
            and not torch.is_grad_enabled() and len(blocks) >= 2 and x.shape[1] == 64 and x.shape[0] > 0):
        return False
    for i, b in enumerate(blocks):
        cin = 64 if i == 0 else 256
        if tuple(b["w1"].shape) != (64, cin, 1, 1) or tuple(b["w2"].shape) != (64, 64, 3, 3) or tuple(b["w3"].shape) != (256, 64, 1, 1):
            return False
        if (b["ws"] is not None) != (i == 0) or (i == 0 and tuple(b["ws"].shape) != (256, 64, 1, 1)):
            return False
        if any(b[k] is not None and (b[k].dtype != torch.float32 or b[k].device != x.device) for k in b):
            return False
    return bool(native.lib().dvis_bneck_x3_supported(1, x.shape[2], x.shape[3]))


def bneck_stage_x3(x, blocks, xexp=None):
    N, _, H, W = x.shape
    lib = native.lib()
    xe = X3_CONV_XEXP if xexp is None else xexp
    dev = x.device

    def packed_conv1():
        w = blocks[0]["w1"]

        return _x3_cache(w, [w], lambda: _x3_pack_conv1x1(w.detach().reshape(64, 64).contiguous()), kind="conv1x1")

    def packed_block(i):
        b, nxt = blocks[i], (blocks[i + 1] if i + 1 < len(blocks) else None)
        ws, w1n = b["ws"], (None if nxt is None else nxt["w1"])

        def make():
            w2 = b["w2"].detach().contiguous()
            w3 = b["w3"].detach().reshape(256, 64).contiguous()
            wsd = None if ws is None else ws.detach().reshape(256, 64).contiguous()
            w1d = None if w1n is None else w1n.detach().reshape(64, 256).contiguous()
            e2, e1 = _x3_wexp(w2), (0 if w1d is None else _x3_wexp(w1d))
            e3 = _x3_wexp(w3 if wsd is None else torch.cat([w3, wsd], 1))
            buf = torch.empty(lib.dvis_bneck_x3_packed_bytes(0 if w1d is None else 1, 0 if wsd is None else 1), dtype=torch.uint8, device=dev)
            with torch.cuda.device(dev):
                native.check(lib.dvis_bneck_x3_pack(native.dev_ptr(w2, "w2"), native.dev_ptr(w3, "w3"),
                                                    None if wsd is None else native.dev_ptr(wsd, "ws"),
                                                    None if w1d is None else native.dev_ptr(w1d, "w1"), e2, e3, e1,
                                                    ctypes.c_void_p(buf.data_ptr()), native.stream_ptr(dev)), "dvis_bneck_x3_pack")
            b3 = b["b3"]
            if b["bs"] is not None:
                b3 = b["bs"].detach() if b3 is None else b3.detach() + b["bs"].detach()
            return buf, e2, e3, e1, (None if b3 is None else b3.detach().clone())
        return _x3_cache(b["w2"], [b["w2"], b["w3"], ws, w1n, b["b3"], b["bs"]], make, kind="bottleneck chain")

    img_bytes = lib.dvis_bneck_x3_image_bytes(N, H, W)
    imgs = [torch.empty(img_bytes, dtype=torch.uint8, device=dev) for _ in range(2)]
    ys = [torch.empty((N, 256, H, W), dtype=torch.float32, device=dev) for _ in range(min(2, len(blocks)))]
    step = max(1, min(N, (2 ** 31 - 1) // (256 * H * W * 4)))
    per_img = img_bytes // N

    def ptr(t):
        return None if t is None else native.dev_ptr(t.detach(), "shift")

    with torch.cuda.device(dev):
        for i0 in range(0, N, step):
            n = min(step, N - i0)
            isl = slice(i0 * per_img, (i0 + n) * per_img)
            buf1, e1 = packed_conv1()
            native.check(lib.dvis_conv1x1_x3_image(native.dev_ptr(x[i0:i0 + n], "x"), ctypes.c_void_p(buf1.data_ptr()), ptr(blocks[0]["b1"]),
                                                   ctypes.c_void_p(imgs[0][isl].data_ptr()), n, 64, H, W, xe, e1, xe, 1, native.stream_ptr(dev)),
                         "dvis_conv1x1_x3_image")
            for i, b in enumerate(blocks):
                buf, e2, e3, e1n, b3 = packed_block(i)
                last = i + 1 == len(blocks)
                y, yprev = ys[i % 2], ys[(i + 1) % 2]
                native.check(lib.dvis_bneck_x3(
                    ctypes.c_void_p(imgs[i % 2][isl].data_ptr()), None if i == 0 else native.dev_ptr(yprev[i0:i0 + n], "res"),
                    native.dev_ptr(x[i0:i0 + n], "x") if i == 0 else None, ctypes.c_void_p(buf.data_ptr()), ptr(b["b2"]), ptr(b3),
                    None if last else ptr(blocks[i + 1]["b1"]), native.dev_ptr(y[i0:i0 + n], "y"),
                    None if last else ctypes.c_void_p(imgs[(i + 1) % 2][isl].data_ptr()), n, H, W, xe, e2, e3, e1n, native.stream_ptr(dev)),
                    "dvis_bneck_x3")
    return ys[(len(blocks) - 1) % 2]


def _fp32_pack(weight, kind, numel, pack, name):
    def make():
        w = weight.detach().contiguous()
        uf = torch.empty(numel, dtype=torch.float32, device=w.device)
        with torch.cuda.device(w.device):
            native.check(pack(native.dev_ptr(w, "weight"), native.dev_ptr(uf, "uf"), native.stream_ptr(w.device)), name)
        return uf
    return derived.TABLE.get(weight, kind, [weight], make)


CONV1X1_MFMA = os.environ.get("DVIS_CONV1X1_MFMA", "1") != "0"


def conv1x1s2_supported(x, weight):
    N, Ci, H, W = x.shape
    return CONV1X1_MFMA and x.is_cuda and x.dtype == torch.float32 and x.is_contiguous() and not torch.is_grad_enabled() \
        and bool(native.lib().dvis_conv1x1_mfma_supported(Ci, weight.shape[0], ((H + 1) // 2) * ((W + 1) // 2))) \
        and 2 * Ci * H * W * 4 < 2 ** 31


def conv1x1_mfma(x, weight, bias=None, res=None, relu=False, stride=1):
    N, Ci, H, W = x.shape
    Co = weight.shape[0]
    uf = _fp32_pack(weight, "conv1x1 mfma", Co * Ci, lambda w, uf, st: native.lib().dvis_conv1x1_mfma_pack(w, uf, Co, Ci, st),
                    "dvis_conv1x1_mfma_pack")
    if stride == 2:
        out = torch.empty((N, Co, (H + 1) // 2, (W + 1) // 2), dtype=torch.float32, device=x.device)
        with torch.cuda.device(x.device):
            rc = native.lib().dvis_conv1x1s2_mfma(
                native.dev_ptr(x, "x"), native.dev_ptr(uf, "uf"), None if bias is None else native.dev_ptr(bias.detach(), "bias"),
                None if res is None else native.dev_ptr(res, "res"), native.dev_ptr(out, "out"), N, Ci, Co, H, W, 1 if relu else 0,
                native.stream_ptr(x.device))
        native.check(rc, "dvis_conv1x1s2_mfma")
        return out
    out = torch.empty((N, Co, H, W), dtype=torch.float32, device=x.device)
    with torch.cuda.device(x.device):
        rc = native.lib().dvis_conv1x1_mfma(
            native.dev_ptr(x, "x"), native.dev_ptr(uf, "uf"), None if bias is None else native.dev_ptr(bias.detach(), "bias"),
            None if res is None else native.dev_ptr(res, "res"), native.dev_ptr(out, "out"), N, Ci, Co, H * W, 1 if relu else 0,
            native.stream_ptr(x.device))
    native.check(rc, "dvis_conv1x1_mfma")
    return out


WINOGRAD_DEFAULT = os.environ.get("DVIS_WINOGRAD", "1") != "0"


def _winograd_weights(weight):
    K, C = weight.shape[:2]
    return _fp32_pack(weight, "winograd", 16 * K * C, lambda w, uf, st: native.lib().dvis_conv3x3_winograd_pack(w, uf, K, C, st),
                      "dvis_conv3x3_winograd_pack")


S2_DEFAULT = os.environ.get("DVIS_CONV3X3S2", "1") != "0"


def _s2_weights(weight):
    K, C = weight.shape[:2]
    return _fp32_pack(weight, "conv3x3s2", 12 * K * C, lambda w, uf, st: native.lib().dvis_conv3x3s2_pack(w, uf, K, C, st),
                      "dvis_conv3x3s2_pack")


def conv3x3s2_bias_act(x, weight, bias=None, relu=False, own=None):
    N, C, H, W = x.shape
    K = weight.shape[0]
    if own is None and conv3x3_x3_ok(x, weight, 2):
        return conv3x3_x3(x, weight, bias, None, relu, 2)
    ok = x.is_cuda and x.dtype == torch.float32 and weight.dtype == torch.float32 and tuple(weight.shape[1:]) == (C, 3, 3) \
        and not (torch.is_grad_enabled() and (x.requires_grad or weight.requires_grad)) \
# ... 617 lines not shown
```

dvis_plus_amd/native.py:

```python
import ctypes
import os

import torch

_HERE = os.path.dirname(os.path.abspath(__file__))
LIB_PATH = os.environ.get("DVIS_HIP_LIB") or os.path.join(_HERE, "lib", "libdvis_hip.so")

F32, F64, F16, BF16 = 0, 1, 2, 3
_DTYPE = {torch.float32: F32, torch.float64: F64, torch.float16: F16, torch.bfloat16: BF16}

_c = ctypes
_i, _i64, _p, _f = _c.c_int, _c.c_int64, _c.c_void_p, _c.c_float

SIGNATURES = {
    "dvis_last_error": (_c.c_char_p, []),
    "dvis_version": (_i, []),
    "dvis_msda_forward": (_i, [_i, _p, _p, _p, _p, _p, _i, _i, _i, _i, _i, _i, _i, _p, _p]),
    "dvis_msda_backward": (_i, [_i, _p, _p, _p, _p, _p, _p, _i, _i, _i, _i, _i, _i, _i, _p, _p, _p, _p]),
    "dvis_msda_backward_det_ws_bytes": (_i64, [_i, _i, _i, _i]),
    "dvis_msda_backward_det": (_i, [_p, _p, _p, _p, _p, _p, _i, _i, _i, _i, _i, _i, _i, _p, _p, _p, _p, _p]),
    "dvis_msda_fused_forward": (_i, [_p, _p, _p, _p, _i, _p, _i64, _p, _i64, _i, _i, _i, _i, _i, _i, _i, _p, _p, _p]),
    "dvis_msda_fused_forward_pos": (_i, [_p, _p, _p, _p, _i, _p, _i64, _p, _i64, _p, _p, _i64, _i, _i, _i, _i, _i, _i, _i,
                                         _p, _p, _p]),
    "dvis_msda_fused_forward_h": (_i, [_i, _p, _p, _p, _p, _i, _p, _i64, _p, _i64, _i, _i, _i, _i, _i, _i, _i, _p, _p, _p]),
    "dvis_msda_fused_forward_slots": (_i, [_p, _p, _p, _p, _i, _p, _i64, _p, _i64, _i, _i, _i, _p, _p, _i64, _i, _i, _i, _i,
                                           _i, _i, _i, _p, _p, _p]),
    "dvis_nchw_to_tokens": (_i, [_p, _p, _i64, _i, _i64, _i64, _i64, _p]),
    "dvis_tokens_to_nchw": (_i, [_p, _p, _i64, _i, _i64, _i64, _i64, _p]),
    "dvis_normalize_pad": (_i, [_p, _i, _p, _i64, _i, _i, _i, _i, _i, _p, _p, _p]),
    "dvis_nchw_to_tokens_affine": (_i, [_p, _p, _p, _p, _p, _p, _i64, _i, _i64, _i64, _i64, _p]),
    "dvis_mask_logits": (_i, [_p, _p, _i, _i, _i, _i64, _p, _p]),
    "dvis_mask_logits_backward_ws_bytes": (_i64, [_i, _i, _i, _i64]),
    "dvis_mask_logits_backward": (_i, [_p, _p, _i, _i, _i, _i64, _p, _p, _p, _p]),
    "dvis_attn_mask": (_i, [_p, _p, _i, _i, _i, _i, _i, _i, _i, _p, _p, _p]),
    "dvis_center_pool3": (_i, [_p, _i64, _i, _i, _p, _p, _p, _p]),
    "dvis_attn_mask_pooled": (_i, [_p, _p, _i, _i, _i, _i, _i, _p, _p, _p]),
    "dvis_attention_ws_bytes": (_i64, [_i, _i, _i, _i]),
    "dvis_attention_ws_bytes_k": (_i64, [_i, _i, _i, _i, _i]),
    "dvis_attention_plan": (_i, [_i, _i, _i, _i, _i, _i64, _i64, _i, _p]),
    "dvis_attention_forward": (_i, [_p, _p, _p, _p, _p, _p, _p, _p, _p, _p, _i, _i, _i, _i, _i, _f, _p, _p]),
    "dvis_attention_forward_k": (_i, [_p, _p, _p, _p, _p, _p, _p, _p, _p, _p, _i, _i, _i, _i, _i, _f, _p, _p, _i]),
    "dvis_attention_backward": (_i, [_p, _p, _p, _p, _p, _p, _p, _p, _p, _p, _p, _i, _i, _i, _i, _i, _f, _p]),
    "dvis_attention_backward_threads": (_i, [_i]),
    "dvis_add_layernorm": (_i, [_p, _p, _i64, _p, _p, _p, _i64, _i, _f, _p]),
    "dvis_add_layernorm_pos": (_i, [_p, _p, _i64, _p, _p, _p, _p, _i64, _p, _i64, _i, _f, _p]),
    "dvis_bias_act": (_i, [_p, _p, _p, _i64, _i, _i64, _i, _p]),
    "dvis_conv3x3_winograd_supported": (_i, [_i, _i, _i, _i]),
    "dvis_conv3x3_winograd_pack": (_i, [_p, _p, _i, _i, _p]),
    "dvis_conv3x3_winograd": (_i, [_p, _p, _p, _p, _i, _i, _i, _i, _i, _i, _p]),
    "dvis_conv3x3s2_supported": (_i, [_i, _i, _i, _i]),
    "dvis_conv3x3s2_pack": (_i, [_p, _p, _i, _i, _p]),
    "dvis_conv3x3s2": (_i, [_p, _p, _p, _p, _i, _i, _i, _i, _i, _i, _p]),
    "dvis_conv7x7s2_supported": (_i, [_i, _i, _i, _i]),
    "dvis_conv7x7s2_pack": (_i, [_p, _p, _p]),
    "dvis_conv7x7s2": (_i, [_p, _p, _p, _p, _i, _i, _i, _i, _p]),
    "dvis_conv1x1_mfma_supported": (_i, [_i, _i, _i64]),
    "dvis_conv1x1_mfma_pack": (_i, [_p, _p, _i, _i, _p]),
    "dvis_conv1x1_mfma": (_i, [_p, _p, _p, _p, _p, _i, _i, _i, _i64, _i, _p]),
    "dvis_conv1x1s2_mfma": (_i, [_p, _p, _p, _p, _p, _i, _i, _i, _i, _i, _i, _p]),
    "dvis_conv1x1_supported": (_i, [_i, _i, _i64]),
    "dvis_conv1x1_bias_act": (_i, [_p, _p, _p, _p, _p, _i, _i, _i, _i64, _i, _p]),
    "dvis_bias_relu_maxpool": (_i, [_p, _p, _p, _i64, _i, _i, _i, _p]),
    "dvis_group_norm_affine": (_i, [_p, _p, _p, _p, _p, _i64, _i, _i, _i64, _f, _p]),
    "dvis_scale_shift_act": (_i, [_p, _p, _p, _i64, _i64, _i, _p]),
    "dvis_upsample_add_affine": (_i, [_p, _p, _p, _p, _p, _i64, _i, _i, _i, _i, _p]),
    "dvis_upsample_add": (_i, [_p, _p, _p, _i64, _i, _i, _i, _i, _p]),
    "dvis_dwconv3x3_tokens": (_i, [_p, _p, _i64, _i, _i, _i, _i, _p, _p, _i, _p]),
    "dvis_adapter_res2": (_i, [_p, _p, _p, _p, _p, _p, _i, _i, _i, _i, _p]),
    "dvis_vps_argmax": (_i, [_p, _i64, _i64, _p, _i, _i, _i, _i, _i, _i, _i, _i, _i, _i, _p, _p, _p, _p]),
    "dvis_vss_argmax": (_i, [_p, _i64, _i64, _p, _i, _i, _i, _i, _i, _i, _i, _i, _i, _i, _i, _i, _p, _p]),
    "dvis_resize2_gt0": (_i, [_p, _i64, _i64, _i, _i, _i, _i, _i, _i, _i, _i, _i, _i, _p, _p]),
    "dvis_resize2": (_i, [_p, _i64, _i64, _i, _i, _i, _i, _i, _i, _i, _i, _i, _i, _i, _p, _p]),
    "dvis_lsap_solve": (_i, [_p, _i, _i, _p]),
    "dvis_match_chain": (_i, [_p, _i, _i, _p]),
    "dvis_gemm_nt": (_i, [_p, _i64, _i64, _p, _i64, _i64, _p, _p, _i64, _i64, _p, _i64, _i64, _i, _i, _i, _i, _i, _i, _p]),
    "dvis_gemm_nt_hm": (_i, [_p, _i64, _i64, _p, _i64, _i64, _p, _p, _i64, _i64, _p, _i64, _i64, _i, _i, _i, _i, _i, _i, _i,
                             _i64, _p]),
    "dvis_gemm_nt_bb": (_i, [_p, _i64, _i64, _p, _i64, _i64, _p, _i64, _p, _i64, _i64, _p, _i64, _i64, _i, _i, _i, _i, _i, _i,
                             _p]),
    "dvis_gemm_ln": (_i, [_p, _i64, _p, _i64, _p, _p, _f, _p, _p, _f, _p, _i64, _p, _i64, _p, _p, _i64, _p, _i64, _i, _i, _i,
                          _i, _i, _p]),
    "dvis_gemm_ln_supported": (_i, [_i, _i, _i, _i]),
    "dvis_gemm_ln_num_configs": (_i, []),
    "dvis_gemm_ln_pick_config": (_i, [_i, _i, _i]),
    "dvis_x3_packed_bytes": (_i64, [_i, _i]),
    "dvis_x3_set_reserve": (_i, [_i]),
    "dvis_x3_set_range_flag": (_i, [_p]),
    "dvis_x3_set_tag": (_i, [_i]),
    "dvis_x3_pack": (_i, [_p, _i64, _i, _i, _i, _p, _p]),
    "dvis_x3_linear_supported": (_i, [_i, _i, _i]),
    "dvis_x3_linear": (_i, [_p, _i64, _i64, _i, _p, _i, _i, _i, _p, _i, _p, _i64, _p]),
    "dvis_x3_tile_supported": (_i, [_i, _i]),
    "dvis_x3_tile_packed_bytes": (_i64, [_i, _i]),
    "dvis_x3_tile_pack": (_i, [_p, _i64, _i, _i, _i, _p, _p]),
    "dvis_x3_tile_linear_qkv": (_i, [_p, _i64, _i64, _i, _p, _i, _i, _i, _p, _i, _i, _f, _p, _p]),
    "dvis_attention_x3_packed": (_i, [_p, _p, _p, _i, _i, _i, _p]),
    "dvis_x3_rows_image_bytes": (_i64, [_i64, _i]),
    "dvis_x3_rows_image": (_i, [_p, _i64, _i64, _i, _i, _p, _p]),
    "dvis_layernorm_rows_image": (_i, [_p, _p, _p, _i64, _i, _f, _i, _p, _p]),
    "dvis_x3_tile_pack_order": (_i, [_p, _i64, _i, _i, _i, _i, _p, _p]),
    "dvis_x3_tile_linear_image": (_i, [_p, _i64, _i, _p, _i, _i, _i, _p, _i, _p, _i64, _p, _i64, _p, _i, _p]),
    "dvis_x3_tile_linear_qkv_image": (_i, [_p, _i64, _i, _p, _i, _i, _i, _p, _i, _i, _f, _p, _p]),
    "dvis_attention_x3_packed_image": (_i, [_p, _p, _i, _i, _i, _i, _p]),
    "dvis_x3_tile_linear": (_i, [_p, _i64, _i64, _i, _p, _i, _i, _i, _p, _i, _p, _i64, _p, _i64, _p]),
    "dvis_x3_linear_res": (_i, [_p, _i64, _i64, _i, _p, _i, _i, _i, _p, _i, _p, _i64, _p, _i64, _p]),
    "dvis_x3_linear_add": (_i, [_p, _i64, _i64, _i, _p, _i, _i, _i, _p, _i64, _p, _i, _p, _i64, _p]),
    "dvis_x3_linear_ln": (_i, [_p, _i64, _i64, _i, _p, _i, _i, _i, _p, _p, _i64, _p, _p, _f, _p, _i64, _p, _p, _i64, _p]),
    "dvis_x3_ffn_packed_bytes": (_i64, [_i, _i, _i]),
    "dvis_x3_ffn_pack": (_i, [_p, _i64, _p, _i64, _i, _i, _i, _i, _i, _p, _p]),
    "dvis_x3_ffn_ln": (_i, [_p, _i64, _i64, _i, _i, _i, _p, _i, _i, _i, _i, _p, _p, _p, _p, _f, _p, _i64, _p, _p, _i64, _p]),
    "dvis_conv1x1_x3_supported": (_i, [_i, _i, _i64, _i64, _i64]),
    "dvis_conv1x1_x3_packed_bytes": (_i64, [_i, _i]),
    "dvis_conv1x1_x3_pack": (_i, [_p, _i, _i, _i, _p, _p]),
    "dvis_conv1x1_x3": (_i, [_p, _p, _p, _p, _p, _i, _i, _i, _i, _i, _i, _i, _i, _i, _p]),
    "dvis_conv1x1_x3_dual": (_i, [_p, _p, _p, _p, _p, _p, _i, _i, _i, _i, _i, _i, _i, _i, _i, _i, _i, _i, _p]),
    "dvis_conv3x3_x3_packed_bytes": (_i64, [_i, _i]),
    "dvis_conv3x3_x3_pack": (_i, [_p, _i, _i, _i, _p, _p]),
    "dvis_conv3x3_x3": (_i, [_p, _p, _p, _p, _p, _i, _i, _i, _i, _i, _i, _i, _i, _i, _p]),
    "dvis_bneck_x3_supported": (_i, [_i64, _i, _i]),
    "dvis_bneck_x3_image_bytes": (_i64, [_i64, _i, _i]),
    "dvis_bneck_x3_packed_bytes": (_i64, [_i, _i]),
    "dvis_bneck_x3_pack": (_i, [_p, _p, _p, _p, _i, _i, _i, _p, _p]),
    "dvis_bneck_x3": (_i, [_p, _p, _p, _p, _p, _p, _p, _p, _p, _i, _i, _i, _i, _i, _i, _i, _p]),
    "dvis_conv1x1_x3_image": (_i, [_p, _p, _p, _p, _i, _i, _i, _i, _i, _i, _i, _i, _p]),
    "dvis_conv_x3_image_bytes": (_i64, [_i64, _i, _i, _i]),
    "dvis_conv_x3_pack_image": (_i, [_p, _i, _i, _i, _i, _p, _p]),
    "dvis_conv_x3_image": (_i, [_p, _p, _p, _p, _p, _p, _p, _i, _i, _i, _i, _i, _i, _i, _i, _i, _i, _i, _p]),
    "dvis_upsample_add_image": (_i, [_p, _p, _p, _p, _p, _i, _i, _i, _i, _i, _i, _i, _p]),
    "dvis_gemm_num_configs": (_i, []),
    "dvis_gemm_pick_config": (_i, [_i, _i, _i, _i]),
    "dvis_gemm_pick_config_nw": (_i, [_i, _i, _i, _i, _i]),
    "dvis_gemm_config_waves": (_i, [_i]),
    "dvis_pan_pair_hist": (_i, [_p, _p, _p, _i, _i, _i, _i64, _p, _p, _p]),
    "dvis_sem_confusion": (_i, [_p, _p, _i64, _i, _p, _p, _p]),
    "dvis_video_consistency": (_i, [_p, _p, _i, _i64, _p, _i, _p, _p, _p]),
    "dvis_rle_encode": (_i, [_p, _i64, _i, _i, _i, _p, _p, _p, _p, _p, _p, _p]),
    "dvis_rle_strings": (_i, [_p, _p, _i64, _p, _p, _p, _p]),
    "dvis_rle_decode": (_i, [_p, _p, _i64, _i, _i, _p, _p]),
    "dvis_track_intersections": (_i, [_p, _i64, _i, _p, _i64, _i, _i, _i64, _i, _p, _p]),
    "dvis_pan_segment_stats": (_i, [_p, _i, _i, _i, _i, _p, _p, _p]),
    "dvis_pan_paint_rgb": (_i, [_p, _i64, _p, _i, _p, _p]),
    "dvis_sem_paint": (_i, [_p, _i64, _p, _p, _p, _p]),
    "dvis_resize_frames_u8": (_i, [_p, _i, _i, _i, _p, _i, _i, _p, _i, _p, _i, _i, _p]),
    "dvis_match_cost_ws_bytes": (_i64, [_i, _i, _i, _i]),
    "dvis_match_cost": (_i, [_p, _p, _i, _p, _p, _p, _i, _i, _i, _i, _i, _i, _i, _i, _i, _f, _f, _f, _p, _p, _p, _p]),
    "dvis_point_sample_rows": (_i, [_p, _i, _p, _i64, _i, _i, _i, _p, _p]),
    "dvis_point_loss_ws_bytes": (_i64, [_i64]),
    "dvis_point_loss_fwd": (_i, [_p, _p, _i, _p, _i, _i, _i, _i, _i, _i, _p, _p, _p]),
    "dvis_point_loss_bwd": (_i, [_p, _p, _i, _p, _p, _p, _p, _i, _i, _i, _i, _i, _i, _f, _p, _p, _p]),
}

_lib = None


def lib():
    global _lib
    if _lib is None:
        if not os.path.exists(LIB_PATH):
            raise RuntimeError(
                f"{LIB_PATH} not found: build it with `python -m dvis_plus_amd.build` "
                "(__graft_entry__.build()).  dvis_plus_amd has no CPU/eager fallback.")
        l = ctypes.CDLL(LIB_PATH)
        for name, (res, args) in SIGNATURES.items():
            fn = getattr(l, name)
            fn.restype, fn.argtypes = res, args
        _lib = l
    return _lib


def check(rc, what):
    if rc != 0:
        msg = lib().dvis_last_error().decode()
        raise RuntimeError(f"{what} failed (code {rc}): {msg}")


def dtype_code(t):
    try:
        return _DTYPE[t.dtype]
    except KeyError:
        raise RuntimeError(f"unsupported dtype {t.dtype}") from None


def dev_ptr(t, name):
    if not t.is_cuda:
        raise RuntimeError(f"{name} must be a GPU tensor (dvis_plus_amd has no CPU path); got device {t.device}")
    if not t.is_contiguous():
        raise RuntimeError(f"{name} tensor has to be contiguous")
    return ctypes.c_void_p(t.data_ptr())


def stream_ptr(device=None):
    return ctypes.c_void_p(torch.cuda.current_stream(device).cuda_stream)
```

dvis_plus_amd/pixel_decoder.py:

```python
import math
import os
import warnings

import torch
import torch.nn.functional as F
from torch import nn
from torch.nn.init import constant_, normal_, xavier_uniform_

from . import derived, functions as Fn
from .d2 import configurable
from .registry import SEM_SEG_HEADS_REGISTRY, ShapeSpec

_POS_IN_KERNEL = os.environ.get("DVIS_MSDA_POS", "0") == "1"
_MSDA_SLOTS = int(os.environ.get("DVIS_MSDA_SLOTS", "0") or 0)
_MSDA_HM = os.environ.get("DVIS_MSDA_HM", "0") == "1"


def _is_power_of_2(n):
    if (not isinstance(n, int)) or (n < 0):
        raise ValueError("invalid input for _is_power_of_2: {} (type: {})".format(n, type(n)))
    return (n & (n - 1) == 0) and n != 0


class PositionEmbeddingSine(nn.Module):
# ... 179 lines not shown
        else:
            output = Fn.MSDeformAttnFunction.apply(value.contiguous(), input_spatial_shapes, input_level_start_index,
                                                   sampling_locations.contiguous(), attention_weights.contiguous(),
                                                   self.im2col_step)
        return self.output_proj(output)


class MSDeformAttnTransformerEncoderLayer(nn.Module):
    def __init__(self, d_model=256, d_ffn=1024, dropout=0.1, activation="relu", n_levels=4, n_heads=8, n_points=4):
        super().__init__()
        if activation != "relu":
            raise NotImplementedError("only relu is used by the DVIS++ configs")
        self.self_attn = MSDeformAttn(d_model, n_levels, n_heads, n_points)
        self.norm1 = nn.LayerNorm(d_model)
        self.linear1 = nn.Linear(d_model, d_ffn)
        self.linear2 = nn.Linear(d_ffn, d_model)
        self.norm2 = nn.LayerNorm(d_model)
        self.dropout_p = dropout

    def pos_in_projection(self, src, pos):
        a = self.self_attn
        return bool(Fn.x3_on() and pos is not None and pos.dim() == 3 and pos.shape[0] == 1 and src.dim() == 3 and src.is_cuda
                    and src.dtype == torch.float32 and not torch.is_grad_enabled() and not torch.is_autocast_enabled()
                    and not _POS_IN_KERNEL and not _MSDA_SLOTS and not _MSDA_HM and a.d_model == 256
                    and 3 * a.n_heads * a.n_levels * a.n_points in (128, 192, 256, 288) and a.d_model // a.n_heads in (32, 64)
                    and (a.n_levels, a.n_points) in ((1, 4), (3, 4), (4, 4)))

    def forward(self, src, pos, reference_points, spatial_shapes, level_start_index, padding_mask=None,
                shapes_py=None, query=None, emit_next_query=False):
        pos_in_proj = self.pos_in_projection(src, pos)
        if query is not None and not pos_in_proj:
            src = self.self_attn(query, reference_points, src, spatial_shapes, level_start_index, padding_mask,
                                 spatial_shapes_py=shapes_py, post=(src, self.norm1))
        else:
            src = self.self_attn(src, reference_points, src, spatial_shapes, level_start_index, padding_mask,
                                 spatial_shapes_py=shapes_py, query_pos=pos, post=(src, self.norm1))
        if Fn.x3_on() and Fn.x3_ffn_ok(src, self.linear1, self.linear2) and self.norm2.weight is not None:
            with_pos = emit_next_query and pos is not None and pos.shape[0] == 1 and src.dim() == 3 and not pos_in_proj
            r = Fn.x3_ffn_ln(src, self.linear1, self.linear2, self.norm2, pos=pos if with_pos else None)
            return r if with_pos or not emit_next_query else (r, None)
        src2 = Fn.linear(Fn.linear_relu(src, self.linear1, tall=True), self.linear2.weight, self.linear2.bias, tall=True)
        if emit_next_query and pos is not None and pos.shape[0] == 1:
            return Fn.add_layer_norm(src2, src, self.norm2, pos=pos)
        out = Fn.add_layer_norm(src2, src, self.norm2)
        return (out, None) if emit_next_query else out


class MSDeformAttnTransformerEncoder(nn.Module):
    def __init__(self, encoder_layer_factory, num_layers):
        super().__init__()
        self.layers = nn.ModuleList([encoder_layer_factory() for _ in range(num_layers)])
        self.num_layers = num_layers
        self._ref_cache = {}

    @staticmethod
    def get_reference_points(spatial_shapes, valid_ratios, device):
        pts = []
        for lvl, (H_, W_) in enumerate(spatial_shapes):
            H_, W_ = int(H_), int(W_)
            ref_y, ref_x = torch.meshgrid(torch.linspace(0.5, H_ - 0.5, H_, dtype=torch.float32, device=device),
                                          torch.linspace(0.5, W_ - 0.5, W_, dtype=torch.float32, device=device),
                                          indexing="ij")
            ref_y = ref_y.reshape(-1)[None] / (valid_ratios[:, None, lvl, 1] * H_)
            ref_x = ref_x.reshape(-1)[None] / (valid_ratios[:, None, lvl, 0] * W_)
            pts.append(torch.stack((ref_x, ref_y), -1))
        reference_points = torch.cat(pts, 1)
        return reference_points[:, :, None] * valid_ratios[:, None]

    def reference_points_unpadded(self, shapes_py, device):
        key = (tuple(shapes_py), str(device))
        if key not in self._ref_cache:
            vr = torch.ones(1, len(shapes_py), 2, device=device)
            self._ref_cache[key] = self.get_reference_points(shapes_py, vr, device).contiguous()
        return self._ref_cache[key]

    def forward(self, src, spatial_shapes, level_start_index, valid_ratios=None, pos=None, padding_mask=None,
                shapes_py=None, query0=None):
        if valid_ratios is None:
            reference_points = self.reference_points_unpadded(shapes_py, src.device)
        else:
            reference_points = self.get_reference_points(spatial_shapes.tolist(), valid_ratios, src.device)
        output, query = src, query0
        for i, layer in enumerate(self.layers):
            last = i + 1 == len(self.layers)
            r = layer(output, pos, reference_points, spatial_shapes, level_start_index, padding_mask,
                      shapes_py=shapes_py, query=query, emit_next_query=not last)
            output, query = (r, None) if last else r
        return output


class MSDeformAttnTransformerEncoderOnly(nn.Module):
    def __init__(self, d_model=256, nhead=8, num_encoder_layers=6, dim_feedforward=1024, dropout=0.1,
                 activation="relu", num_feature_levels=4, enc_n_points=4):
        super().__init__()
        self.d_model, self.nhead = d_model, nhead
        self.encoder = MSDeformAttnTransformerEncoder(
            lambda: MSDeformAttnTransformerEncoderLayer(d_model, dim_feedforward, dropout, activation,
                                                        num_feature_levels, nhead, enc_n_points),
            num_encoder_layers)
        self.level_embed = nn.Parameter(torch.Tensor(num_feature_levels, d_model))
        self._shape_cache = {}
        self._reset_parameters()

    def _reset_parameters(self):
        for p in self.parameters():
            if p.dim() > 1:
                nn.init.xavier_uniform_(p)
        for m in self.modules():
            if isinstance(m, MSDeformAttn):
                m._reset_parameters()
        normal_(self.level_embed)

    def _shape_tensors(self, shapes_py, device):
        key = (tuple(shapes_py), str(device))
        if key not in self._shape_cache:
            s = torch.as_tensor(shapes_py, dtype=torch.long, device=device)
            lsi = torch.cat((s.new_zeros((1,)), s.prod(1).cumsum(0)[:-1]))
            self._shape_cache[key] = (s, lsi)
        return self._shape_cache[key]

    def forward(self, srcs, pos_embeds, affines=None):
        shapes_py = [(int(s.shape[2]), int(s.shape[3])) for s in srcs]
        lvl_pos = torch.cat([p.flatten(2).transpose(1, 2) + self.level_embed[lvl].view(1, 1, -1)
                             for lvl, p in enumerate(pos_embeds)], 1)
        query0 = None
        layer0 = self.encoder.layers[0] if len(self.encoder.layers) else None
        probe = srcs[0].new_empty((1, 1, srcs[0].shape[1]))
        if layer0 is not None and layer0.pos_in_projection(probe, lvl_pos):
            src_flatten = Fn.maps_to_tokens(srcs, affines)
        elif lvl_pos.shape[0] == 1 and srcs[0].is_cuda and not torch.is_grad_enabled():
            src_flatten, query0 = Fn.maps_to_tokens(srcs, affines, pos=lvl_pos)
        else:
            src_flatten = Fn.maps_to_tokens(srcs, affines)
        spatial_shapes, level_start_index = self._shape_tensors(shapes_py, src_flatten.device)
        memory = self.encoder(src_flatten, spatial_shapes, level_start_index, None, lvl_pos, None, shapes_py=shapes_py,
                              query0=query0)
        return memory, spatial_shapes, level_start_index, shapes_py


class ConvNorm(nn.Conv2d):

    def __init__(self, *args, norm=None, activation=None, **kwargs):
        super().__init__(*args, **kwargs)
        self.norm, self.activation = norm, activation

    def conv(self, x):
        if self.kernel_size == (1, 1) and self.stride == (1, 1) and self.groups == 1 and self.padding == (0, 0):
            return Fn.conv1x1(x, self.weight, self.bias)
        if self.kernel_size == (3, 3) and self.stride == (1, 1) and self.padding == (1, 1) and self.dilation == (1, 1) \
                and self.groups == 1 and x.is_cuda and not torch.is_grad_enabled():
            return Fn.conv3x3_bias_act(x, self.weight, self.bias)
        return F.conv2d(x, self.weight, self.bias, self.stride, self.padding, self.dilation, self.groups)

    def conv_and_affine(self, x):
        if isinstance(self.norm, nn.GroupNorm) and self.activation is None:
            y = self.conv(x)
            aff = Fn.group_norm_affine(y, self.norm)
            if aff is not None:
                return y, aff
            return self.norm(y), None
        return self.forward(x), None

    def image_input_ok(self, N, C, H, W, device):
        return self.stride == (1, 1) and self.dilation == (1, 1) and self.groups == 1 and self.weight.dtype == torch.float32 \
            and ((self.kernel_size == (3, 3) and self.padding == (1, 1)) or (self.kernel_size == (1, 1) and self.padding == (0, 0))) \
            and C == self.in_channels and Fn.x3_images_ok(N, C, self.out_channels, H, W, device, taps=self.kernel_size[0] ** 2)

    def forward(self, x):
        if isinstance(x, Fn.OperandImage):
            x = Fn.conv_x3_image(x, self.weight, self.bias)
        else:
            x = self.conv(x)
        if isinstance(self.norm, nn.GroupNorm) and self.activation in (None, F.relu):
            aff = Fn.group_norm_affine(x, self.norm)
            if aff is not None:
                return Fn.scale_shift_act_(x, aff[0], aff[1], relu=self.activation is not None)
        if self.norm is not None:
            x = self.norm(x)
        if self.activation is not None:
            x = self.activation(x)
        return x


def get_norm(norm, out_channels):
    if norm is None or norm == "":
        return None
    if norm != "GN":
        raise NotImplementedError(f"norm {norm!r}: the DVIS++ configs use GN")
    return nn.GroupNorm(32, out_channels)


def c2_xavier_fill(module):
    nn.init.kaiming_uniform_(module.weight, a=1)
    if module.bias is not None:
        nn.init.constant_(module.bias, 0)


@SEM_SEG_HEADS_REGISTRY.register()
class MSDeformAttnPixelDecoder(nn.Module):
    @configurable
    def __init__(self, input_shape, *, transformer_dropout, transformer_nheads, transformer_dim_feedforward,
                 transformer_enc_layers, conv_dim, mask_dim, norm=None, transformer_in_features, common_stride):
        super().__init__()
        transformer_input_shape = {k: v for k, v in input_shape.items() if k in transformer_in_features}
        input_shape = sorted(input_shape.items(), key=lambda x: x[1].stride)
        self.in_features = [k for k, v in input_shape]
        self.feature_strides = [v.stride for k, v in input_shape]
        self.feature_channels = [v.channels for k, v in input_shape]
        transformer_input_shape = sorted(transformer_input_shape.items(), key=lambda x: x[1].stride)
        self.transformer_in_features = [k for k, v in transformer_input_shape]
        transformer_in_channels = [v.channels for k, v in transformer_input_shape]
        self.transformer_feature_strides = [v.stride for k, v in transformer_input_shape]
        self.transformer_num_feature_levels = len(self.transformer_in_features)
        chans = transformer_in_channels[::-1] if self.transformer_num_feature_levels > 1 \
            else [transformer_in_channels[-1]]
        self.input_proj = nn.ModuleList([
            nn.Sequential(nn.Conv2d(c, conv_dim, kernel_size=1), nn.GroupNorm(32, conv_dim)) for c in chans])
        for proj in self.input_proj:
            nn.init.xavier_uniform_(proj[0].weight, gain=1)
            nn.init.constant_(proj[0].bias, 0)
        self.transformer = MSDeformAttnTransformerEncoderOnly(
            d_model=conv_dim, dropout=transformer_dropout, nhead=transformer_nheads,
            dim_feedforward=transformer_dim_feedforward, num_encoder_layers=transformer_enc_layers,
            num_feature_levels=self.transformer_num_feature_levels)
        self.pe_layer = PositionEmbeddingSine(conv_dim // 2, normalize=True)
        self.mask_dim = mask_dim
        self.mask_features = ConvNorm(conv_dim, mask_dim, kernel_size=1, stride=1, padding=0)
        c2_xavier_fill(self.mask_features)
        self.maskformer_num_feature_levels = 3
        self.common_stride = common_stride
        stride = min(self.transformer_feature_strides)
        self.num_fpn_levels = int(math.log2(stride) - math.log2(self.common_stride))
        lateral_convs, output_convs = [], []
        use_bias = norm == ""
        for idx, in_channels in enumerate(self.feature_channels[:self.num_fpn_levels]):
            lateral_conv = ConvNorm(in_channels, conv_dim, kernel_size=1, bias=use_bias, norm=get_norm(norm, conv_dim))
            output_conv = ConvNorm(conv_dim, conv_dim, kernel_size=3, stride=1, padding=1, bias=use_bias,
                                   norm=get_norm(norm, conv_dim), activation=F.relu)
            c2_xavier_fill(lateral_conv)
            c2_xavier_fill(output_conv)
            self.add_module("adapter_{}".format(idx + 1), lateral_conv)
            self.add_module("layer_{}".format(idx + 1), output_conv)
            lateral_convs.append(lateral_conv)
            output_convs.append(output_conv)
        self.lateral_convs = lateral_convs[::-1]
        self.output_convs = output_convs[::-1]

    @classmethod
    def from_config(cls, cfg, input_shape):
        hd = cfg.MODEL.SEM_SEG_HEAD
        return dict(
            input_shape={k: v for k, v in input_shape.items() if k in hd.IN_FEATURES},
            conv_dim=hd.CONVS_DIM, mask_dim=hd.MASK_DIM, norm=hd.NORM,
            transformer_dropout=cfg.MODEL.MASK_FORMER.DROPOUT, transformer_nheads=cfg.MODEL.MASK_FORMER.NHEADS,
            transformer_dim_feedforward=1024, transformer_enc_layers=hd.TRANSFORMER_ENC_LAYERS,
            transformer_in_features=hd.DEFORMABLE_TRANSFORMER_ENCODER_IN_FEATURES, common_stride=hd.COMMON_STRIDE)

    def forward_features(self, features):
        with torch.autocast(device_type="cuda", enabled=False), Fn.x3_stage("pd_proj"):
            srcs, pos, affines = [], [], []
            for idx, f in enumerate(self.transformer_in_features[::-1]):
                x = features[f].float().contiguous()
                conv, gn = self.input_proj[idx][0], self.input_proj[idx][1]
                s_ = Fn.conv1x1(x, conv.weight, conv.bias) if conv.kernel_size == (1, 1) and conv.stride == (1, 1) \
                    and conv.padding == (0, 0) and conv.groups == 1 else conv(x)
                affine = Fn.group_norm_affine(s_, gn)
                srcs.append(s_ if affine is not None else gn(s_))
                affines.append(affine)
                pos.append(self.pe_layer.compute(x.shape[2], x.shape[3], x.device))
            with Fn.x3_stage("encoder"):
                y, _, _, shapes_py = self.transformer(srcs, pos, affines)
            bs = y.shape[0]
            out, tokens, start = [], [], 0
            for li, (h, w) in enumerate(shapes_py):
                tokens.append(y[:, start:start + h * w])
                if li + 1 == len(shapes_py) and self.num_fpn_levels > 0:
                    out.append(Fn.tokens_to_map(y, start, h, w))
                else:
                    out.append(tokens[-1].transpose(1, 2).reshape(bs, -1, h, w))
                start += h * w
            with Fn.x3_stage("mask_path"):
                for idx, f in enumerate(self.in_features[:self.num_fpn_levels][::-1]):
                    x = features[f].float().contiguous()
                    cur_fpn, affine = self.lateral_convs[idx].conv_and_affine(x)
                    oc = self.output_convs[idx]
                    if cur_fpn.is_cuda and cur_fpn.dtype == torch.float32 and cur_fpn.is_contiguous() and out[-1].dtype == torch.float32 \
                            and oc.image_input_ok(*cur_fpn.shape, cur_fpn.device):
                        out.append(oc(Fn.upsample_add_image(cur_fpn, out[-1], affine)))
                    else:
                        out.append(oc(Fn.upsample_add(cur_fpn, out[-1], affine)))
                multi_scale_features = TokenMaps(out[:self.maskformer_num_feature_levels])
                multi_scale_features.tokens = tokens[:self.maskformer_num_feature_levels]
                return self.mask_features(out[-1]), out[0], multi_scale_features


class TokenMaps(list):
    tokens = None


def r50_input_shape():
    return {"res2": ShapeSpec(channels=256, stride=4), "res3": ShapeSpec(channels=512, stride=8),
            "res4": ShapeSpec(channels=1024, stride=16), "res5": ShapeSpec(channels=2048, stride=32)}
```

include/dvis_hip.h:

```cpp
#ifndef DVIS_HIP_H
#define DVIS_HIP_H

#include <stdint.h>

#ifdef __cplusplus
extern "C" {
#endif

enum { DVIS_F32 = 0, DVIS_F64 = 1, DVIS_F16 = 2, DVIS_BF16 = 3 };

enum {
  DVIS_OK = 0,
  DVIS_E_ARG = -1,
  DVIS_E_LAUNCH = -2,
  DVIS_E_UNSUPPORTED = -3
};

const char *dvis_last_error(void);
int dvis_version(void);

int dvis_msda_forward(int dtype, const void *value, const int64_t *shapes, const int64_t *level_start,
                      const void *loc, const void *w, int N, int S, int M, int D, int L, int Lq, int P,
                      void *out, void *stream);

int dvis_msda_backward(int dtype, const void *value, const int64_t *shapes, const int64_t *level_start,
                       const void *loc, const void *w, const void *grad_out,
                       int N, int S, int M, int D, int L, int Lq, int P,
                       void *grad_value, void *grad_loc, void *grad_w, void *stream);

int64_t dvis_msda_backward_det_ws_bytes(int N, int S, int M, int D);
int dvis_msda_backward_det(const float *value, const int64_t *shapes, const int64_t *level_start, const float *loc, const float *w,
                           const float *grad_out, int N, int S, int M, int D, int L, int Lq, int P, float *grad_value, float *grad_loc,
                           float *grad_w, void *ws, void *stream);

int dvis_msda_fused_forward(const float *value, const int64_t *shapes, const int64_t *level_start,
                            const float *ref, int Nref, const float *offsets, int64_t off_stride,
                            const float *logits, int64_t logit_stride,
                            int N, int S, int M, int D, int L, int Lq, int P, float *out,
                            const int64_t *shapes_host, void *stream);

int dvis_msda_fused_forward_pos(const float *value, const int64_t *shapes, const int64_t *level_start,
                                const float *ref, int Nref, const float *offsets, int64_t off_stride,
                                const float *logits, int64_t logit_stride, const float *pos_offsets,
                                const float *pos_logits, int64_t pos_stride, int N, int S, int M, int D, int L, int Lq,
                                int P, float *out, const int64_t *shapes_host, void *stream);

int dvis_msda_fused_forward_h(int dtype, const void *value, const int64_t *shapes, const int64_t *level_start,
                              const float *ref, int Nref, const void *offsets, int64_t off_stride, const void *logits,
                              int64_t logit_stride, int N, int S, int M, int D, int L, int Lq, int P, void *out,
                              const int64_t *shapes_host, void *stream);

int dvis_msda_fused_forward_slots(const float *value, const int64_t *shapes, const int64_t *level_start,
                                  const float *ref, int Nref, const float *offsets, int64_t off_stride,
                                  const float *logits, int64_t logit_stride, int off_head_stride, int logit_head_stride,
                                  int value_head_major, const float *pos_offsets, const float *pos_logits, int64_t pos_stride, int N, int S,
                                  int M, int D, int L, int Lq, int P, float *out, const int64_t *shapes_host,
                                  void *stream);

int dvis_mask_logits(const float *embed, const float *feat, int B, int Q, int C, int64_t HW,
                     float *out, void *stream);

int64_t dvis_mask_logits_backward_ws_bytes(int B, int R, int C, int64_t HW);
int dvis_mask_logits_backward(const float *g, const float *feat, int B, int R, int C, int64_t HW, float *grad_embed,
                              float *row_sum, void *ws, void *stream);

int dvis_attn_mask(const float *embed, const float *feat, int B, int Q, int C, int H, int W, int h, int w,
                   uint8_t *mask, int32_t *allowed_count, void *stream);
int dvis_center_pool3(const float *feat, int64_t planes, int H, int W, float *p2, float *p4, float *p8, void *stream);
int dvis_attn_mask_pooled(const float *embed, const float *pooled, int B, int Q, int C, int h, int w, uint8_t *mask,
                          int32_t *allowed_count, void *stream);

int64_t dvis_attention_ws_bytes(int BH, int Lq, int Lk, int d);
int dvis_attention_forward(const float *q, const int64_t *q_strides, const float *k, const int64_t *k_strides,
                           const float *v, const int64_t *v_strides, float *out, const int64_t *o_strides,
                           const uint8_t *mask, const int32_t *allowed_count, int B, int heads, int Lq, int Lk,
                           int d, float scale, void *ws, void *stream);
int dvis_attention_forward_k(const float *q, const int64_t *q_strides, const float *k, const int64_t *k_strides,
                           const float *v, const int64_t *v_strides, float *out, const int64_t *o_strides,
                           const uint8_t *mask, const int32_t *allowed_count, int B, int heads, int Lq, int Lk,
                           int d, float scale, void *ws, void *stream, int kernel);
int64_t dvis_attention_ws_bytes_k(int BH, int Lq, int Lk, int d, int kernel);
enum {
  DVIS_ATTN_FWD = 0,
  DVIS_ATTN_SHORT = 1,
  DVIS_ATTN_X3 = 2,
  DVIS_ATTN_KEYSPLIT = 3
};
int dvis_attention_plan(int BH, int Lq, int Lk, int d, int has_mask, int64_t k_row, int64_t v_row, int kernel, int32_t *plan);

int dvis_attention_backward(const float *q, const int64_t *q_strides, const float *k, const int64_t *k_strides,
                            const float *v, const int64_t *v_strides, const float *grad_out, const int64_t *g_strides,
                            float *dq, float *dk, float *dv, int B, int heads, int Lq, int Lk, int d, float scale,
                            void *stream);
int dvis_attention_backward_threads(int Lk);

int dvis_add_layernorm(const float *x, const float *res, int64_t res_row_stride, const float *gamma, const float *beta,
                       float *out, int64_t rows, int C, float eps, void *stream);

int dvis_add_layernorm_pos(const float *x, const float *res, int64_t res_row_stride, const float *gamma, const float *beta,
                           float *out, const float *pos, int64_t pos_rows, float *out_pos, int64_t rows, int C, float eps,
                           void *stream);

int dvis_upsample_add(const float *lateral, const float *top, float *out, int64_t planes, int H, int W, int h, int w,
                      void *stream);

int dvis_nchw_to_tokens(const float *x, float *out, int64_t N, int C, int64_t HW, int64_t S, int64_t row0, void *stream);

int dvis_tokens_to_nchw(const float *tok, float *out, int64_t N, int C, int64_t HW, int64_t S, int64_t row0, void *stream);
int dvis_normalize_pad(const void *in, int is_u8, float *out, int64_t planes, int C, int H, int W, int Hp, int Wp, const float *mean,
                       const float *stdv, void *stream);
int dvis_nchw_to_tokens_affine(const float *x, const float *scale, const float *shift, const float *pos, float *out,
                               float *out_pos, int64_t N, int C, int64_t HW, int64_t S, int64_t row0, void *stream);

int dvis_conv1x1_supported(int K, int M, int64_t HW);
int dvis_conv1x1_mfma_supported(int C, int K, int64_t HW);
int dvis_conv1x1_mfma_pack(const float *w, float *uf, int K, int C, void *stream);
int dvis_conv1x1_mfma(const float *x, const float *uf, const float *bias, const float *res, float *y, int N, int C, int K, int64_t HW,
                      int relu, void *stream);
int dvis_conv1x1s2_mfma(const float *x, const float *uf, const float *bias, const float *res, float *y, int N, int C, int K, int H, int W,
                        int relu, void *stream);
int dvis_conv1x1_bias_act(const float *x, const float *w, const float *bias, const float *res, float *out,
                          int N, int K, int M, int64_t HW, int relu, void *stream);

int dvis_conv3x3_winograd_supported(int C, int K, int H, int W);
int dvis_conv3x3s2_supported(int C, int K, int H, int W);
int dvis_conv7x7s2_supported(int C, int K, int H, int W);
int dvis_conv7x7s2_pack(const float *w, float *uf, void *stream);
int dvis_conv7x7s2(const float *x, const float *uf, const float *bias, float *y, int N, int H, int W, int relu, void *stream);
int dvis_conv3x3s2_pack(const float *w, float *uf, int K, int C, void *stream);
int dvis_conv3x3s2(const float *x, const float *uf, const float *bias, float *y, int N, int C, int K, int H, int W, int relu,
                   void *stream);
int dvis_conv3x3_winograd_pack(const float *w, float *uf, int K, int C, void *stream);
int dvis_conv3x3_winograd(const float *x, const float *uf, const float *bias, float *y, int N, int C, int K, int H, int W,
                          int relu, void *stream);

int dvis_bias_act(float *x, const float *bias, const float *res, int64_t planes, int C, int64_t HW, int relu,
                  void *stream);

int dvis_bias_relu_maxpool(const float *x, const float *bias, float *out, int64_t planes, int C, int H, int W,
                           void *stream);

int dvis_group_norm_affine(const float *x, const float *gamma, const float *beta, float *scale, float *shift, int64_t N,
                           int C, int G, int64_t HW, float eps, void *stream);
int dvis_scale_shift_act(float *x, const float *scale, const float *shift, int64_t planes, int64_t HW, int relu,
                         void *stream);
int dvis_upsample_add_affine(const float *lateral, const float *lat_scale, const float *lat_shift, const float *top,
                             float *out, int64_t planes, int H, int W, int h, int w, void *stream);

int dvis_dwconv3x3_tokens(const float *x, float *out, int64_t batch_stride, int B, int h, int w, int C, const float *weight,
                          const float *bias, int gelu, void *stream);

int dvis_adapter_res2(const float *g, const float *c1, const float *x1, const float *scale, const float *shift, float *out, int B, int C,
                      int h8, int w8, void *stream);

int dvis_vps_argmax(const float *logits, int64_t stride_k, int64_t stride_t, const float *scores, int K, int T,
                    int h, int w, int first_h, int first_w, int img_h, int img_w, int out_h, int out_w,
                    int32_t *ids, uint8_t *conf, int32_t *areas, void *stream);

int dvis_resize2_gt0(const float *logits, int64_t stride_k, int64_t stride_t, int K, int T, int h, int w, int first_h,
                     int first_w, int img_h, int img_w, int out_h, int out_w, uint8_t *out, void *stream);

int dvis_resize2(const float *logits, int64_t stride_k, int64_t stride_t, int K, int T, int h, int w, int first_h,
                 int first_w, int img_h, int img_w, int out_h, int out_w, int sigmoid, float *out, void *stream);

int dvis_vss_argmax(const float *logits, int64_t stride_q, int64_t stride_t, const float *cls, int cls_row_stride, int Q,
                    int C, int T, int h, int w, int first_h, int first_w, int img_h, int img_w, int out_h, int out_w,
                    int64_t *out, void *stream);

int dvis_lsap_solve(const double *cost, int nr, int nc, int64_t *col4row);

int dvis_match_chain(const float *cost, int T, int Q, int64_t *indices);

int dvis_gemm_nt(const float *A, int64_t lda, int64_t strideA, const float *W, int64_t ldw, int64_t strideW,
                 const float *bias, const float *res, int64_t ldres, int64_t strideRes, float *C, int64_t ldc,
                 int64_t strideC, int M, int N, int K, int batch, int act, int config, void *stream);
int dvis_gemm_nt_hm(const float *A, int64_t lda, int64_t strideA, const float *W, int64_t ldw, int64_t strideW,
                    const float *bias, const float *res, int64_t ldres, int64_t strideRes, float *C, int64_t ldc,
                    int64_t strideC, int M, int N, int K, int batch, int act, int config, int head_d, int64_t head_stride,
                    void *stream);
int dvis_gemm_nt_bb(const float *A, int64_t lda, int64_t strideA, const float *W, int64_t ldw, int64_t strideW,
                    const float *bias, int64_t strideBias, const float *res, int64_t ldres, int64_t strideRes, float *C,
                    int64_t ldc, int64_t strideC, int M, int N, int K, int batch, int act, int config, void *stream);
int dvis_gemm_num_configs(void);
int dvis_gemm_pick_config(int M, int N, int K, int batch);
int dvis_gemm_pick_config_nw(int M, int N, int K, int batch, int nw);
int dvis_gemm_config_waves(int config);

int dvis_gemm_ln(const float *A, int64_t lda, const float *add, int64_t ldadd, const float *gamma1, const float *beta1,
                 float eps1, const float *gamma2, const float *beta2, float eps2, float *a_out, int64_t ldaout,
                 const float *W, int64_t ldw, const float *bias, const float *res, int64_t ldres, float *C, int64_t ldc,
                 int M, int N, int K, int act, int config, void *stream);
int dvis_gemm_ln_supported(int M, int N, int K, int norms);
int dvis_gemm_ln_num_configs(void);
int dvis_gemm_ln_pick_config(int M, int N, int K);

int64_t dvis_x3_packed_bytes(int N, int K);
int dvis_x3_set_reserve(int cus);
int dvis_x3_set_range_flag(int32_t *device_word);
int dvis_x3_set_tag(int tag);
int dvis_x3_pack(const float *W, int64_t ldw, int N, int K, int wexp, void *packed, void *stream);
int dvis_x3_linear_supported(int N, int K, int ln);
int dvis_x3_linear(const float *x, int64_t ldx, int64_t M, int K, const void *packed, int N, int xexp, int wexp,
                   const float *bias, int relu, float *out, int64_t ldo, void *stream);
int dvis_x3_linear_add(const float *x, int64_t ldx, int64_t M, int K, const void *packed, int N, int xexp, int wexp,
                       const float *xadd, int64_t xadd_rows, const float *bias, int relu, float *out, int64_t ldo, void *stream);
int dvis_x3_linear_res(const float *x, int64_t ldx, int64_t M, int K, const void *wp, int N, int xexp, int wexp, const float *bias, int act,
                       const float *res, int64_t ldres, float *out, int64_t ldo, void *stream);

int dvis_x3_tile_supported(int N, int K);
int64_t dvis_x3_tile_packed_bytes(int N, int K);
int dvis_x3_tile_pack(const float *w, int64_t ldw, int N, int K, int wexp, void *packed, void *stream);
int dvis_x3_tile_linear(const float *x, int64_t ldx, int64_t M, int K, const void *wp, int N, int xexp, int wexp, const float *bias, int act,
                        const float *res, int64_t ldres, float *out, int64_t ldo, void *stream);
int dvis_x3_tile_linear_qkv(const float *x, int64_t ldx, int64_t M, int K, const void *wp, int N, int xexp, int wexp, const float *bias,
                            int heads, int L, float qscale, void *ws, void *stream);
int dvis_attention_x3_packed(const void *ws, float *out, const int64_t *o_strides, int B, int heads, int L, void *stream);
int64_t dvis_x3_rows_image_bytes(int64_t M, int K);
int dvis_x3_rows_image(const float *x, int64_t ldx, int64_t M, int K, int xexp, void *image, void *stream);
int dvis_layernorm_rows_image(const float *x, const float *gamma, const float *beta, int64_t M, int C, float eps, int xexp, void *image,
                              void *stream);
int dvis_x3_tile_pack_order(const float *w, int64_t ldw, int N, int K, int wexp, int order, void *packed, void *stream);
int dvis_x3_tile_linear_image(const void *ximg, int64_t M, int K, const void *wp, int N, int xexp, int wexp, const float *bias, int act,
                              const float *res, int64_t ldres, float *out, int64_t ldo, void *oimg, int oexp, void *stream);
int dvis_x3_tile_linear_qkv_image(const void *ximg, int64_t M, int K, const void *wp, int N, int xexp, int wexp, const float *bias, int heads,
                                  int L, float qscale, void *ws, void *stream);
int dvis_attention_x3_packed_image(const void *ws, void *image, int B, int heads, int L, int xexp, void *stream);
int dvis_x3_linear_ln(const float *x, int64_t ldx, int64_t M, int K, const void *packed, int N, int xexp, int wexp,
                      const float *bias, const float *res, int64_t ldres, const float *gamma, const float *beta, float eps,
                      const float *pos, int64_t pos_rows, float *out, float *out2, int64_t ldo, void *stream);
int64_t dvis_x3_ffn_packed_bytes(int K, int H, int N);
int dvis_conv1x1_x3_supported(int C, int K, int64_t N, int64_t HW_in, int64_t HW_out);
int64_t dvis_conv1x1_x3_packed_bytes(int C, int K);
int dvis_conv1x1_x3_pack(const float *w, int K, int C, int wexp, void *packed, void *stream);
int dvis_conv1x1_x3(const float *x, const void *packed, const float *bias, const float *res, float *y, int N, int C, int K, int H,
                    int W, int stride, int xexp, int wexp, int relu, void *stream);
int dvis_conv1x1_x3_dual(const float *x, const float *x2, const void *packed, const float *bias, const float *res, float *y, int N,
                         int C, int C2, int K, int H, int W, int H2, int W2, int stride2, int xexp, int wexp, int relu, void *stream);
int64_t dvis_conv3x3_x3_packed_bytes(int C, int K);
int dvis_conv3x3_x3_pack(const float *w, int K, int C, int wexp, void *packed, void *stream);
int dvis_conv3x3_x3(const float *x, const void *packed, const float *bias, const float *res, float *y, int N, int C, int K, int H,
                    int W, int stride, int xexp, int wexp, int relu, void *stream);
int dvis_bneck_x3_supported(int64_t N, int H, int W);
int64_t dvis_bneck_x3_image_bytes(int64_t N, int H, int W);
int64_t dvis_bneck_x3_packed_bytes(int tail, int dual);
int dvis_bneck_x3_pack(const float *w2, const float *w3, const float *ws, const float *w1, int e2, int e3, int e1, void *packed,
                       void *stream);
int dvis_bneck_x3(const void *a1, const float *res, const float *x2, const void *packed, const float *b2, const float *b3,
                  const float *b1, float *y, void *out, int N, int H, int W, int xexp, int e2, int e3, int e1, void *stream);
int dvis_conv1x1_x3_image(const float *x, const void *packed, const float *bias, void *image, int N, int C, int H, int W, int xexp,
                          int wexp, int oexp, int relu, void *stream);
int64_t dvis_conv_x3_image_bytes(int64_t N, int C, int H, int W);
int dvis_conv_x3_pack_image(const float *w, int K, int C, int taps, int wexp, void *packed, void *stream);
int dvis_conv_x3_image(const void *ximg, const float *x, const void *packed, const float *bias, const float *res, float *y, void *image,
                       int N, int C, int K, int H, int W, int stride, int taps, int xexp, int wexp, int oexp, int relu, void *stream);
int dvis_upsample_add_image(const float *lateral, const float *lat_scale, const float *lat_shift, const float *top, void *image, int N,
                            int C, int H, int W, int h, int w, int oexp, void *stream);
int dvis_x3_ffn_pack(const float *W1, int64_t ldw1, const float *W2, int64_t ldw2, int K, int H, int N, int w1exp, int w2exp,
                     void *packed, void *stream);
int dvis_x3_ffn_ln(const float *x, int64_t ldx, int64_t M, int K, int H, int N, const void *packed, int xexp, int w1exp,
                   int hexp, int w2exp, const float *b1, const float *b2, const float *gamma, const float *beta, float eps,
                   const float *pos, int64_t pos_rows, float *out, float *out2, int64_t ldo, void *stream);

int dvis_pan_pair_hist(const int32_t *gt, const int32_t *pred, const int32_t *gt_table, int Ng, int Np, int T, int64_t HW,
                       int64_t *out, int64_t *bad, void *stream);
int dvis_sem_confusion(const int32_t *gt, const int32_t *pred, int64_t n, int num_class, int64_t *out, int64_t *bad, void *stream);
int dvis_video_consistency(const int32_t *gt, const int32_t *pred, int T, int64_t HW, const int32_t *ks, int nk, int64_t *gt_const,
                           int64_t *both_const, void *stream);

int dvis_rle_encode(const uint8_t *masks, int64_t N, int H, int W, int phase, int64_t *trans, int64_t *area, const int64_t *toff,
                    const int64_t *moff, int32_t *bnd, uint32_t *runs, void *stream);
int dvis_rle_strings(const uint32_t *runs, const int64_t *run_off, int64_t N, const int64_t *str_off, int64_t *lens, uint8_t *chars,
                     void *stream);
int dvis_rle_decode(const int32_t *ends, const int64_t *run_off, int64_t N, int H, int W, uint8_t *out, void *stream);
int dvis_track_intersections(const uint8_t *pred, int64_t pred_stride, int P, const uint8_t *gt, int64_t gt_stride, int G, int T,
                             int64_t HW, int accumulate, int64_t *out, void *stream);

int dvis_pan_segment_stats(const int32_t *map, int T, int H, int W, int n, int64_t *out, int64_t *bad, void *stream);
int dvis_pan_paint_rgb(const int32_t *map, int64_t npx, const int32_t *lut, int nlut, uint8_t *out, void *stream);
int dvis_sem_paint(const int32_t *map, int64_t npx, const int32_t *lut, uint8_t *out, int64_t *bad, void *stream);

int dvis_resize_frames_u8(const uint8_t *in, int T, int H, int W, uint8_t *out, int h, int w, const int32_t *xtab, int kx,
                          const int32_t *ytab, int ky, int reverse, void *stream);

int64_t dvis_match_cost_ws_bytes(int Q, int G, int T, int K);
int dvis_match_cost(const float *pred, const void *tgt, int tgt_u8, const float *coords, const float *logits,
                    const int64_t *tgt_ids, int Q, int G, int T, int H, int W, int Ht, int Wt, int K, int NC, float w_class,
                    float w_mask, float w_dice, float *C, float *terms, void *ws, void *stream);
int dvis_point_sample_rows(const void *rows, int rows_u8, const float *coords, int64_t R, int P, int H, int W, float *out,
                           void *stream);
int64_t dvis_point_loss_ws_bytes(int64_t R);
int dvis_point_loss_fwd(const float *src, const void *tgt, int tgt_u8, const float *coords, int R, int P, int H, int W, int Ht, int Wt,
                        float *out, void *ws, void *stream);
int dvis_point_loss_bwd(const float *src, const void *tgt, int tgt_u8, const float *coords, const float *sums, const float *g_mask,
                        const float *g_dice, int R, int P, int H, int W, int Ht, int Wt, float num_masks, float *grad_src,
                        void *det_ws, void *stream);

#ifdef __cplusplus
}
#endif
#endif
```

Baseline: 411.8.

## Fuse GroupNorm statistics into conv epilogue and GN affine into next conv input

Adds optional extras to the x3 conv kernel. The epilogue can emit fp64 per-32-pixel, per-8-channel partial sums and squared sums for GroupNorm, which a new finalize kernel reduces to scale and shift. The 1x1 path can also apply a per-sample scale, shift and ReLU to its fp32 input from an LDS table, instead of running a separate scale_shift_act pass. This removes separate reads of the conv output for GN statistics and the normalize pass before mask_features. The cost is extra epilogue shuffles, fp64 arithmetic, per-tile LDS table loads with __syncthreads, and thread-local state passed across API calls.

```diff
diff --git a/dvis_plus_amd/csrc/conv1x1_x3.hip b/dvis_plus_amd/csrc/conv1x1_x3.hip
--- a/dvis_plus_amd/csrc/conv1x1_x3.hip
+++ b/dvis_plus_amd/csrc/conv1x1_x3.hip
@@ -28,6 +28,9 @@
   int OH;
   const void *ximg;
   int XG_in;
+  double *gn_part;
+  const float *in_scale, *in_shift;
+  int in_relu;
 };
 
 __device__ __forceinline__ bool cx_item(const CxArgs &a, long long w, long long *tile, int *pass) {
@@ -77,13 +80,16 @@
   return (unsigned)(n * a.C2 * a.HW2_in * 4) + (unsigned)((oy * a.stride2 * a.W2_in + ox * a.stride2) * 4);
 }
 
-template <int NB, int NW, int IK, bool IMGIN = false, bool IMGOUT = false>
+template <int NB, int NW, int IK, bool IMGIN = false, bool IMGOUT = false, int EXT = 0>
 __global__ __launch_bounds__(NW * 64) void conv1x1_x3_kernel(const CxArgs a) {
+  static_assert(EXT == 0 || (NB == 8 && !IMGOUT), "the extras serve the 256-channel passes with an fp32 output");
+  static_assert(!(EXT & 2) || !IMGIN, "the input affine is applied to an fp32 input");
   constexpr int kTile = NW * 32, PW = 2 * IK * NB / NW, STAGES = IK == 4 ? 2 : 3, IPC = 4 / IK;
   static_assert(2 * IK * NB % NW == 0, "the item's pieces must divide among the waves");
   extern __shared__ __attribute__((aligned(1024))) char lds[];
   const int wave = threadIdx.x >> 6, lane = threadIdx.x & 63, j = lane & 31, g = lane >> 5;
-  const int NCC = a.C / 64, NC1 = a.taps * NCC, NC = NC1 + a.C2 / 64, NI = IPC * NC;
+  constexpr bool kOne = (EXT & 2) != 0;
+  const int NCC = a.C / 64, NC1 = kOne ? NCC : a.taps * NCC, NC = kOne ? NCC : NC1 + a.C2 / 64, NI = IPC * NC;
   long long wcount = 0;
   {
     long long t;
@@ -145,19 +151,44 @@
   long long tile;
   int pass;
   cx_item(a, 0, &tile, &pass);
-  CxGeom gm = cx_geom(a, tile * kTile + wave * 32 + j);
-  unsigned gm2 = cx_geom2(a, tile * kTile + wave * 32 + j);
+  auto geom = [&](long long q) -> CxGeom {
+    if constexpr (kOne) {
+      const long long n = q / a.HW;
+      return CxGeom{q < a.pixels ? (unsigned)((n * a.C * a.HW + (q - n * a.HW)) * 4) : kOOB, 0, 0, 0};
+    } else {
+      return cx_geom(a, q);
+    }
+  };
+  auto tap_offset = [&](const CxGeom &m, int tap) -> unsigned {
+    if constexpr (kOne) return m.base;
+    else return cx_tap_offset(a, m, tap);
+  };
+  CxGeom gm = geom(tile * kTile + wave * 32 + j);
+  unsigned gm2 = kOne ? kOOB : cx_geom2(a, tile * kTile + wave * 32 + j);
   if constexpr (IMGIN)
     load_img(cx_tap_offset_img(a, gm, 0, g), 0);
   else
-    load_raw(cx_tap_offset(a, gm, 0), 0);
+    load_raw(tap_offset(gm, 0), 0);
+  float *const tab = (float *)(lds + STAGES * RingT::kItemBytes);
   for (long long w = 0; w < wcount; ++w) {
     const long long p = tile * kTile + wave * 32 + j;
+    int tsel = 0;
+    if constexpr ((EXT & 2) != 0) {
+      const long long n0 = tile * kTile / a.HW;
+      __syncthreads();
+      for (int i = threadIdx.x; i < 4 * a.C; i += NW * 64) {
+        const int im = i / (2 * a.C), r = i - im * 2 * a.C, c = r < a.C ? r : r - a.C;
+        const long long nn = n0 + im;
+        tab[i] = nn < a.N ? (r < a.C ? a.in_scale : a.in_shift)[nn * a.C + c] : 0.f;
+      }
+      __syncthreads();
+      tsel = p / a.HW > n0 ? 1 : 0;
+    }
     long long ntile = tile;
     int npass_ = pass;
     const bool more = cx_item(a, w + 1, &ntile, &npass_);
-    const CxGeom ngm = more ? cx_geom(a, ntile * kTile + wave * 32 + j) : CxGeom{kOOB, 0, 0, 0};
-    const unsigned ngm2 = more ? cx_geom2(a, ntile * kTile + wave * 32 + j) : kOOB;
+    const CxGeom ngm = more ? geom(ntile * kTile + wave * 32 + j) : CxGeom{kOOB, 0, 0, 0};
+    const unsigned ngm2 = more && !kOne ? cx_geom2(a, ntile * kTile + wave * 32 + j) : kOOB;
     int tap = 0, cc = 0;
     f16v acc[NB];
 #pragma unroll
@@ -182,15 +213,34 @@
       } else {
 #pragma unroll
         for (int i = 0; i < 32; ++i) asm volatile("" : "+v"(raw[i]));
-#pragma unroll
-        for (int s = 0; s < 4; ++s) {
-          const f4 lo4 = {raw[8 * s], raw[8 * s + 1], raw[8 * s + 2], raw[8 * s + 3]};
-          const f4 hi4 = {raw[8 * s + 4], raw[8 * s + 5], raw[8 * s + 6], raw[8 * s + 7]};
-          split8(lo4, hi4, a.xscale, xh[s], xl[s]);
+        if constexpr ((EXT & 2) != 0) {
+          int to = tsel * 2 * a.C + 64 * kc + 8 * g;
+#pragma unroll
+          for (int s = 0; s < 4; ++s) {
+            const float *ts = tab + to;
+            const f4 a0 = *(const f4 *)(ts + 16 * s), a1 = *(const f4 *)(ts + 16 * s + 4);
+            const f4 b0 = *(const f4 *)(ts + a.C + 16 * s), b1 = *(const f4 *)(ts + a.C + 16 * s + 4);
+            f4 lo4, hi4;
+#pragma unroll
+            for (int e = 0; e < 4; ++e) {
+              lo4[e] = raw[8 * s + e] * a0[e] + b0[e], hi4[e] = raw[8 * s + 4 + e] * a1[e] + b1[e];
+              if (a.in_relu) lo4[e] = fmaxf(lo4[e], 0.f), hi4[e] = fmaxf(hi4[e], 0.f);
+            }
+            split8(lo4, hi4, a.xscale, xh[s], xl[s]);
+            asm volatile("" : "+v"(to) : "v"(xh[s]), "v"(xl[s]));
+          }
+          asm volatile("" : "+v"(gm.base), "+v"(tsel) : "v"(to));
+        } else {
+#pragma unroll
+          for (int s = 0; s < 4; ++s) {
+            const f4 lo4 = {raw[8 * s], raw[8 * s + 1], raw[8 * s + 2], raw[8 * s + 3]};
+            const f4 hi4 = {raw[8 * s + 4], raw[8 * s + 5], raw[8 * s + 6], raw[8 * s + 7]};
+            split8(lo4, hi4, a.xscale, xh[s], xl[s]);
+          }
         }
         if (++cc == NCC) cc = 0, ++tap;
-        const bool first = kc + 1 < NC1, sec = !first && kc + 1 < NC;
-        const unsigned po = first ? cx_tap_offset(a, gm, tap) : (sec ? gm2 : cx_tap_offset(a, ngm, 0));
+        const bool first = kc + 1 < NC1, sec = !kOne && !first && kc + 1 < NC;
+        const unsigned po = first ? tap_offset(gm, tap) : (sec ? gm2 : tap_offset(ngm, 0));
         load_raw(po, first ? cc : (sec ? kc + 1 - NC1 : 0), sec);
       }
 #pragma unroll
@@ -247,6 +297,7 @@
         rv[r] = a.res ? __builtin_bit_cast(float, __builtin_amdgcn_raw_buffer_load_b32(
                                                       rr, obase + (unsigned)(co0 + 32 * nb + 8 * (r >> 2) + 4 * g + (r & 3)) * ochan, 0, 0))
                       : 0.f;
+      [[maybe_unused]] double part[8];
 #pragma unroll
       for (int q = 0; q < 4; ++q) {
         const int co = co0 + 32 * nb + 8 * q + 4 * g;
@@ -259,7 +310,28 @@
           chk = __builtin_fmaf(v, 0.f, chk);
           if (a.relu) v = x3_relu(v);
           __builtin_amdgcn_raw_buffer_store_b32(__builtin_bit_cast(unsigned, v), ry, o, 0, 0);
+          if constexpr ((EXT & 1) != 0) rv[4 * q + i] = v;
         }
+        if constexpr ((EXT & 1) != 0) {
+          const double d0 = rv[4 * q], d1 = rv[4 * q + 1], d2 = rv[4 * q + 2], d3 = rv[4 * q + 3];
+          part[2 * q] = (d0 + d1) + (d2 + d3);
+          part[2 * q + 1] = (d0 * d0 + d1 * d1) + (d2 * d2 + d3 * d3);
+        }
+      }
+      if constexpr ((EXT & 1) != 0) {
+        double h4[4], h2[2];
+#pragma unroll
+        for (int k = 0; k < 4; ++k) h4[k] = (g ? part[4 + k] : part[k]) + __shfl_xor(g ? part[k] : part[4 + k], 32);
+        const bool b4 = (lane & 16) != 0, b3 = (lane & 8) != 0;
+#pragma unroll
+        for (int k = 0; k < 2; ++k) h2[k] = (b4 ? h4[2 + k] : h4[k]) + __shfl_xor(b4 ? h4[k] : h4[2 + k], 16);
+        double t = (b3 ? h2[1] : h2[0]) + __shfl_xor(b3 ? h2[0] : h2[1], 8);
+        t += __shfl_xor(t, 4);
+        t += __shfl_xor(t, 2);
+        t += __shfl_xor(t, 1);
+        const long long p0 = p - j;
+        if ((lane & 7) == 0 && p0 < a.pixels)
+          a.gn_part[(((p0 / a.HW) * (a.HW >> 5) + ((p0 % a.HW) >> 5)) * (a.K >> 3) + ((co0 + 32 * nb) >> 3)) * 2 + (lane >> 3)] = t;
       }
     }
     if (a.flag != nullptr && chk != chk && p < a.pixels) atomicCAS(a.flag, 0, a.tag);
@@ -358,9 +430,27 @@
                      int stride, int taps, int xexp, int wexp, int relu, void *stream, const float *x2 = nullptr, int C2 = 0, int H2 = 0,
                      int W2 = 0, int stride2 = 1, void *image = nullptr, int oexp = 0, const void *ximg = nullptr);
 
+struct CxExtras {
+  double *gn_part;
+  const float *in_scale, *in_shift;
+  int in_relu;
+};
+static thread_local CxExtras t_cx_extras = {};
+static thread_local CxExtras t_cx_taken = {};
+struct CxExtrasOnce {
+  CxExtrasOnce() { t_cx_taken = t_cx_extras, t_cx_extras = CxExtras{}; }
+  ~CxExtrasOnce() { t_cx_taken = CxExtras{}; }
+};
+
+DVIS_EXPORT int dvis_conv_x3_set_extras(double *gn_part, const float *in_scale, const float *in_shift, int in_relu) {
+  t_cx_extras = CxExtras{gn_part, in_scale, in_shift, in_relu};
+  return DVIS_OK;
+}
+
 DVIS_EXPORT int dvis_conv1x1_x3_dual(const float *x, const float *x2, const void *packed, const float *bias, const float *res, float *y,
                                      int N, int C, int C2, int K, int H, int W, int H2, int W2, int stride2, int xexp, int wexp, int relu,
                                      void *stream) {
+  const CxExtrasOnce extras;
   DVIS_REQUIRE(x2 != nullptr && C2 >= 64 && C2 % 64 == 0 && C2 <= 4096, "dvis_conv1x1_x3_dual: C2 %% 64 == 0 (got %d)", C2);
   DVIS_REQUIRE((stride2 == 1 || stride2 == 2) && (H2 + stride2 - 1) / stride2 == H && (W2 + stride2 - 1) / stride2 == W,
                "dvis_conv1x1_x3_dual: x2 (%d x %d, stride %d) must down-sample onto x's %d x %d map", H2, W2, stride2, H, W);
@@ -370,11 +460,13 @@
 
 DVIS_EXPORT int dvis_conv1x1_x3(const float *x, const void *packed, const float *bias, const float *res, float *y, int N, int C, int K,
                                 int H, int W, int stride, int xexp, int wexp, int relu, void *stream) {
+  const CxExtrasOnce extras;
   return cx_launch(x, packed, bias, res, y, N, C, K, H, W, stride, 1, xexp, wexp, relu, stream);
 }
 
 DVIS_EXPORT int dvis_conv1x1_x3_image(const float *x, const void *packed, const float *bias, void *image, int N, int C, int H, int W, int xexp,
                                       int wexp, int oexp, int relu, void *stream) {
+  const CxExtrasOnce extras;
   DVIS_REQUIRE(image != nullptr && (uintptr_t)image % 16 == 0, "dvis_conv1x1_x3_image: null / unaligned image");
   DVIS_REQUIRE((long long)N * H * ((W + 31) / 32) * 8192 < ((long long)1 << 31), "dvis_conv1x1_x3_image: the image must stay below 2 GiB");
   return cx_launch(x, packed, bias, nullptr, nullptr, N, C, 64, H, W, 1, 1, xexp, wexp, relu, stream, nullptr, 0, 0, 0, 1, image, oexp);
@@ -400,6 +492,7 @@
 DVIS_EXPORT int dvis_conv_x3_image(const void *ximg, const float *x, const void *packed, const float *bias, const float *res, float *y,
                                    void *image, int N, int C, int K, int H, int W, int stride, int taps, int xexp, int wexp, int oexp, int relu,
                                    void *stream) {
+  const CxExtrasOnce extras;
   DVIS_REQUIRE(ximg != nullptr || image != nullptr, "dvis_conv_x3_image: neither side is an operand image (use dvis_conv1x1_x3 / dvis_conv3x3_x3)");
   DVIS_REQUIRE((ximg != nullptr) != (x != nullptr), "dvis_conv_x3_image: exactly one of ximg and x");
   DVIS_REQUIRE((image != nullptr) != (y != nullptr), "dvis_conv_x3_image: exactly one of image and y");
@@ -431,6 +524,7 @@
 
 DVIS_EXPORT int dvis_conv3x3_x3(const float *x, const void *packed, const float *bias, const float *res, float *y, int N, int C, int K,
                                 int H, int W, int stride, int xexp, int wexp, int relu, void *stream) {
+  const CxExtrasOnce extras;
   return cx_launch(x, packed, bias, res, y, N, C, K, H, W, stride, 9, xexp, wexp, relu, stream);
 }
 
@@ -454,33 +548,49 @@
   a.x2 = x2, a.C2 = x2 ? C2 : 0, a.stride2 = stride2, a.W2_in = W2, a.HW2_in = (long long)H2 * W2;
   a.img = image, a.XG = (OW + 31) / 32, a.oscale = ldexpf(1.f, oexp), a.OH = OH;
   a.ximg = ximg, a.XG_in = (W + 31) / 32;
+  const CxExtras ex = t_cx_taken;
+  const bool gn = ex.gn_part != nullptr, aff = ex.in_scale != nullptr || ex.in_shift != nullptr;
+  if (gn || aff) {
+    DVIS_REQUIRE(!(gn && aff), "dvis_conv_x3_set_extras: partial sums and an input affine in one launch are not served");
+    DVIS_REQUIRE(K % 256 == 0 && y != nullptr && image == nullptr && x2 == nullptr, "dvis_conv_x3_set_extras: K %% 256 == 0 (got %d), an fp32 "
+                 "output map and a single source", K);
+    DVIS_REQUIRE(!gn || (a.HW % 32 == 0 && (uintptr_t)ex.gn_part % 8 == 0), "dvis_conv_x3_set_extras: partial sums need H * W %% 32 == 0 "
+                 "(got %lld)", a.HW);
+    DVIS_REQUIRE(!aff || (ex.in_scale && ex.in_shift && ximg == nullptr && taps == 1 && stride == 1 && C <= 512 && a.HW >= 256),
+                 "dvis_conv_x3_set_extras: the input affine serves 1x1 / stride 1 launches on an fp32 map with C <= 512 and H * W >= 256 "
+                 "(C %d, taps %d, stride %d, H * W %lld)", C, taps, stride, a.HW);
+    a.gn_part = ex.gn_part, a.in_scale = ex.in_scale, a.in_shift = ex.in_shift, a.in_relu = ex.in_relu;
+  }
   const int grid = dvis_x3_persistent_cus();
   hipStream_t st = (hipStream_t)stream;
   static const int nw = getenv("DVIS_X3_CONV_WAVES") ? atoi(getenv("DVIS_X3_CONV_WAVES")) : 8;
   a.npass = K <= 128 ? 1 : K / 256;
-#define DVIS_CX_LAUNCH(NBV, NWV, IKV)                                                                              \
-  {                                                                                                                \
-    static DvisLdsOptIn opted;                                                                                     \
-    typedef Ring<2 * IKV * NBV / NWV, 32, NWV, (IKV == 4 ? 2 : 3)> R;                                              \
-    a.tiles = (a.pixels + 32 * NWV - 1) / (32 * NWV);                                                              \
-    const size_t lds = (IKV == 4 ? 2 : 3) * R::kItemBytes;                                                         \
-    const int rc = dvis_lds_opt_in((const void *)conv1x1_x3_kernel<NBV, NWV, IKV>, lds, &opted, "dvis_conv1x1_x3"); \
-    if (rc != DVIS_OK) return rc;                                                                                  \
-    hipLaunchKernelGGL((conv1x1_x3_kernel<NBV, NWV, IKV>), dim3(grid), dim3(NWV * 64), lds, st, a);                \
-  }
-#define DVIS_CX_LAUNCH_IMG(NBV, IKV, INV, OUTV)                                                                                    \
+#define DVIS_CX_LAUNCH_EXT(NBV, NWV, IKV, EXTV)                                                                                    \
+  {                                                                                                                                \
+    static DvisLdsOptIn opted;                                                                                                     \
+    typedef Ring<2 * IKV * NBV / NWV, 32, NWV, (IKV == 4 ? 2 : 3)> R;                                                              \
+    a.tiles = (a.pixels + 32 * NWV - 1) / (32 * NWV);                                                                              \
+    const size_t lds = (IKV == 4 ? 2 : 3) * R::kItemBytes + (((EXTV) & 2) ? 16 * (size_t)C : 0);                                   \
+    const int rc = dvis_lds_opt_in((const void *)conv1x1_x3_kernel<NBV, NWV, IKV, false, false, EXTV>, lds, &opted, "dvis_conv1x1_x3"); \
+    if (rc != DVIS_OK) return rc;                                                                                                  \
+    hipLaunchKernelGGL((conv1x1_x3_kernel<NBV, NWV, IKV, false, false, EXTV>), dim3(grid), dim3(NWV * 64), lds, st, a);            \
+  }
+#define DVIS_CX_LAUNCH(NBV, NWV, IKV) DVIS_CX_LAUNCH_EXT(NBV, NWV, IKV, 0)
+#define DVIS_CX_LAUNCH_IMG_EXT(NBV, IKV, INV, OUTV, EXTV)                                                                          \
   {                                                                                                                                \
     static DvisLdsOptIn opted;                                                                                                     \
     typedef Ring<2 * IKV * NBV / 8, 8, 8, (IKV == 4 ? 2 : 3)> R;                                                                   \
     a.tiles = (a.pixels + 255) / 256;                                                                                              \
     const size_t lds = (IKV == 4 ? 2 : 3) * R::kItemBytes;                                                                         \
-    const int rc = dvis_lds_opt_in((const void *)conv1x1_x3_kernel<NBV, 8, IKV, INV, OUTV>, lds, &opted, "dvis_conv_x3_image");    \
+    const int rc = dvis_lds_opt_in((const void *)conv1x1_x3_kernel<NBV, 8, IKV, INV, OUTV, EXTV>, lds, &opted, "dvis_conv_x3_image"); \
     if (rc != DVIS_OK) return rc;                                                                                                  \
-    hipLaunchKernelGGL((conv1x1_x3_kernel<NBV, 8, IKV, INV, OUTV>), dim3(grid), dim3(512), lds, st, a);                            \
+    hipLaunchKernelGGL((conv1x1_x3_kernel<NBV, 8, IKV, INV, OUTV, EXTV>), dim3(grid), dim3(512), lds, st, a);                      \
     return dvis_check_launch("dvis_conv_x3_image");                                                                                \
   }
+#define DVIS_CX_LAUNCH_IMG(NBV, IKV, INV, OUTV) DVIS_CX_LAUNCH_IMG_EXT(NBV, IKV, INV, OUTV, 0)
   if (ximg != nullptr || (image != nullptr && K != 64)) {
     DVIS_REQUIRE(x2 == nullptr, "dvis_conv_x3_image: no second source");
+    if (gn) DVIS_CX_LAUNCH_IMG_EXT(8, 4, true, false, 1)
     if (K == 128) {
       if (ximg && image) DVIS_CX_LAUNCH_IMG(4, 2, true, true)
       if (ximg) DVIS_CX_LAUNCH_IMG(4, 2, true, false)
@@ -491,8 +601,13 @@
     DVIS_CX_LAUNCH_IMG(8, 4, false, true)
   }
 #undef DVIS_CX_LAUNCH_IMG
+#undef DVIS_CX_LAUNCH_IMG_EXT
   static const int ik = getenv("DVIS_X3_CONV_ITEM") ? atoi(getenv("DVIS_X3_CONV_ITEM")) : 4;
-  if (K == 64) {
+  if (gn) {
+    DVIS_CX_LAUNCH_EXT(8, 8, 4, 1)
+  } else if (aff) {
+    DVIS_CX_LAUNCH_EXT(8, 8, 4, 2)
+  } else if (K == 64) {
     if (nw == 8) DVIS_CX_LAUNCH(2, 8, 2) else DVIS_CX_LAUNCH(2, 4, 2)
   } else if (K == 128) {
     if (nw == 8) DVIS_CX_LAUNCH(4, 8, 2) else DVIS_CX_LAUNCH(4, 4, 2)
@@ -502,5 +617,6 @@
     if (nw == 8) DVIS_CX_LAUNCH(8, 8, 2) else DVIS_CX_LAUNCH(8, 4, 2)
   }
 #undef DVIS_CX_LAUNCH
+#undef DVIS_CX_LAUNCH_EXT
   return dvis_check_launch("dvis_conv1x1_x3");
 }
diff --git a/dvis_plus_amd/csrc/fused_elementwise.hip b/dvis_plus_amd/csrc/fused_elementwise.hip
--- a/dvis_plus_amd/csrc/fused_elementwise.hip
+++ b/dvis_plus_amd/csrc/fused_elementwise.hip
@@ -657,6 +657,50 @@
   }
 }
 
+__global__ __launch_bounds__(256) void group_norm_finalize_kernel(const double *__restrict__ part, const float *__restrict__ gamma,
+                                                                  const float *__restrict__ beta, float *__restrict__ scale,
+                                                                  float *__restrict__ shift, int C, int G, long long blocks,
+                                                                  float eps) {
+  __shared__ double s_sum[4], s_sq[4];
+  const int Cg = C / G;
+  const int n = blockIdx.x / G, g = blockIdx.x - n * G;
+  const double *pp = part + ((size_t)n * blocks * G + g) * 2;
+  double sum = 0.0, sq = 0.0;
+  for (long long b = threadIdx.x; b < blocks; b += 256) {
+    const double2 v = *reinterpret_cast<const double2 *>(pp + (size_t)b * G * 2);
+    sum += v.x;
+    sq += v.y;
+  }
+#pragma unroll
+  for (int o = 32; o > 0; o >>= 1) {
+    sum += __shfl_down(sum, o);
+    sq += __shfl_down(sq, o);
+  }
+  const int wv = threadIdx.x >> 6;
+  if ((threadIdx.x & 63) == 0) {
+    s_sum[wv] = sum;
+    s_sq[wv] = sq;
+  }
+  __syncthreads();
+  for (int t = threadIdx.x; t < Cg; t += 256) {
+    double ts = 0.0, tq = 0.0;
+#pragma unroll
+    for (int i = 0; i < 4; ++i) {
+      ts += s_sum[i];
+      tq += s_sq[i];
+    }
+    const double count = (double)Cg * 32.0 * (double)blocks;
+    const double mean = ts / count;
+    double var = tq / count - mean * mean;
+    var = var < 0.0 ? 0.0 : var;
+    const float rstd = (float)(1.0 / sqrt(var + (double)eps));
+    const int c = g * Cg + t;
+    const float a = rstd * (gamma ? gamma[c] : 1.f);
+    scale[(size_t)n * C + c] = a;
+    shift[(size_t)n * C + c] = (beta ? beta[c] : 0.f) - (float)mean * a;
+  }
+}
+
 __global__ __launch_bounds__(256) void scale_shift_act_kernel(float *__restrict__ x, const float *__restrict__ scale,
                                                               const float *__restrict__ shift, int HW4, int chunks, int relu) {
   const unsigned plane = blockIdx.x / chunks;
@@ -698,6 +742,17 @@
   return dvis_check_launch("group_norm_affine_kernel");
 }
 
+DVIS_EXPORT int dvis_group_norm_finalize(const double *part, const float *gamma, const float *beta, float *scale, float *shift,
+                                         int64_t N, int C, int G, int64_t blocks, float eps, void *stream) {
+  DVIS_REQUIRE(N >= 0 && C > 0 && G > 0 && blocks > 0 && C % G == 0, "group_norm_finalize: bad sizes (C=%d G=%d)", C, G);
+  if (N == 0) return DVIS_OK;
+  DVIS_REQUIRE(part && scale && shift && ((uintptr_t)part & 15) == 0, "group_norm_finalize: null / unaligned pointer");
+  DVIS_REQUIRE(N * G < (1ll << 31), "group_norm_finalize: too many groups");
+  hipLaunchKernelGGL(group_norm_finalize_kernel, dim3((unsigned)(N * G)), dim3(256), 0, (hipStream_t)stream, part, gamma, beta,
+                     scale, shift, C, G, (long long)blocks, eps);
+  return dvis_check_launch("group_norm_finalize_kernel");
+}
+
 DVIS_EXPORT int dvis_scale_shift_act(float *x, const float *scale, const float *shift, int64_t planes, int64_t HW, int relu,
                                      void *stream) {
   DVIS_REQUIRE(planes >= 0 && HW > 0, "scale_shift_act: bad sizes");
diff --git a/dvis_plus_amd/functions.py b/dvis_plus_amd/functions.py
--- a/dvis_plus_amd/functions.py
+++ b/dvis_plus_amd/functions.py
@@ -700,6 +700,39 @@
     return scale, shift
 
 
+GN_FUSED = os.environ.get("DVIS_GN_FUSED", "1") != "0"
+
+
+def gn_fused_ok(norm, Co, HW):
+    return bool(GN_FUSED and isinstance(norm, torch.nn.GroupNorm) and norm.num_channels == Co and Co % 256 == 0
+                and Co == 8 * norm.num_groups and HW % 32 == 0 and HW > 0)
+
+
+def _gn_partials(N, Co, HW, device):
+    return torch.empty((N, HW // 32, Co // 8, 2), dtype=torch.float64, device=device)
+
+
+def _set_conv_extras(part=None, in_affine=None, in_relu=False):
+    native.check(native.lib().dvis_conv_x3_set_extras(
+        None if part is None else ctypes.c_void_p(part.data_ptr()),
+        None if in_affine is None else native.dev_ptr(in_affine[0], "scale"),
+        None if in_affine is None else native.dev_ptr(in_affine[1], "shift"), 1 if in_relu else 0), "dvis_conv_x3_set_extras")
+
+
+def _gn_finalize(part, norm):
+    N, blocks, G, _ = part.shape
+    C = 8 * G
+    scale = torch.empty(N * C, dtype=torch.float32, device=part.device)
+    shift = torch.empty(N * C, dtype=torch.float32, device=part.device)
+    with torch.cuda.device(part.device):
+        rc = native.lib().dvis_group_norm_finalize(
+            ctypes.c_void_p(part.data_ptr()), None if norm.weight is None else native.dev_ptr(norm.weight.detach(), "gamma"),
+            None if norm.bias is None else native.dev_ptr(norm.bias.detach(), "beta"), native.dev_ptr(scale, "scale"),
+            native.dev_ptr(shift, "shift"), N, C, G, blocks, float(norm.eps), native.stream_ptr(part.device))
+    native.check(rc, "dvis_group_norm_finalize")
+    return scale, shift
+
+
 def scale_shift_act_(x, scale, shift, relu=False):
     N, C, H, W = x.shape
     with torch.cuda.device(x.device):
@@ -1589,7 +1622,23 @@
     return max(1, min(N, (2 ** 31 - 1) // per))
 
 
-def conv1x1_x3(x, weight, bias=None, res=None, relu=False, stride=1, xexp=None):
+def conv1x1_gn(x, weight, bias, norm):
+    if conv1x1_x3_ok(x, weight) and gn_fused_ok(norm, weight.shape[0], x.shape[2] * x.shape[3]) and x.shape[0] > 0:
+        return conv1x1_x3(x, weight, bias, gn=norm)
+    y = conv1x1(x, weight, bias)
+    return y, group_norm_affine(y, norm)
+
+
+def conv1x1_in_affine_ok(x, weight):
+    return bool(GN_FUSED and conv1x1_x3_ok(x, weight) and x.shape[0] > 0 and x.shape[1] <= 512 and weight.shape[0] % 256 == 0
+                and x.shape[2] * x.shape[3] >= 256)
+
+
+def conv1x1_in_affine(x, weight, bias, affine, relu=False):
+    return conv1x1_x3(x, weight, bias, in_affine=affine, in_relu=relu)
+
+
+def conv1x1_x3(x, weight, bias=None, res=None, relu=False, stride=1, xexp=None, gn=None, in_affine=None, in_relu=False):
     N, Ci, H, W = x.shape
     Co = weight.shape[0]
 
@@ -1598,17 +1647,23 @@
     buf, wexp = _x3_cache(weight, [weight], make, kind="conv1x1")
     OH, OW = (H + stride - 1) // stride, (W + stride - 1) // stride
     out = torch.empty((N, Co, OH, OW), dtype=torch.float32, device=x.device)
+    part = None if gn is None else _gn_partials(N, Co, OH * OW, x.device)
+    if in_affine is not None:
+        in_affine = (in_affine[0].reshape(N, Ci), in_affine[1].reshape(N, Ci))
     step = _conv_x3_chunks(N, Ci, Co, H * W, OH * OW)
     with torch.cuda.device(x.device):
         for i in range(0, N, step):
             n = min(step, N - i)
+            if part is not None or in_affine is not None:
+                _set_conv_extras(None if part is None else part[i:i + n],
+                                 None if in_affine is None else (in_affine[0][i:i + n], in_affine[1][i:i + n]), in_relu)
             native.check(native.lib().dvis_conv1x1_x3(
                 native.dev_ptr(x[i:i + n], "x"), ctypes.c_void_p(buf.data_ptr()),
                 None if bias is None else native.dev_ptr(bias.detach(), "bias"),
                 None if res is None else native.dev_ptr(res[i:i + n], "res"), native.dev_ptr(out[i:i + n], "out"), n, Ci, Co, H, W,
                 stride, X3_CONV_XEXP if xexp is None else xexp, wexp, 1 if relu else 0, native.stream_ptr(x.device)),
                 "dvis_conv1x1_x3")
-    return out
+    return out if gn is None else (out, _gn_finalize(part, gn))
 
 
 X3_DUAL = os.environ.get("DVIS_X3_DUAL", "1") != "0"
@@ -1728,7 +1783,7 @@
     return img
 
 
-def conv_x3_image(src, weight, bias=None, res=None, relu=False, stride=1, out_image=False, oexp=None, xexp=None):
+def conv_x3_image(src, weight, bias=None, res=None, relu=False, stride=1, out_image=False, oexp=None, xexp=None, gn=None):
     lib = native.lib()
     from_img = isinstance(src, OperandImage)
     if not (from_img or out_image):
@@ -1752,17 +1807,22 @@
         out = OperandImage(torch.empty(lib.dvis_conv_x3_image_bytes(N, K, OH, OW), dtype=torch.uint8, device=dev), N, K, OH, OW, oe)
     else:
         out = torch.empty((N, K, OH, OW), dtype=torch.float32, device=dev)
+    if gn is not None and out_image:
+        raise ValueError("conv_x3_image: GroupNorm statistics are summed for an fp32 map output")
+    part = None if gn is None else _gn_partials(N, K, OH * OW, dev)
     step = _image_chunks(N, C, K, H, W, OH, OW)
     with torch.cuda.device(dev):
         for i in range(0, N, step):
             n = min(step, N - i)
+            if part is not None:
+                _set_conv_extras(part[i:i + n])
             native.check(lib.dvis_conv_x3_image(
                 ctypes.c_void_p(src.images(i, n).data_ptr()) if from_img else None, None if from_img else native.dev_ptr(src[i:i + n], "x"),
                 ctypes.c_void_p(buf.data_ptr()), None if bias is None else native.dev_ptr(bias.detach(), "bias"),
                 None if res is None else native.dev_ptr(res[i:i + n], "res"), None if out_image else native.dev_ptr(out[i:i + n], "out"),
                 ctypes.c_void_p(out.images(i, n).data_ptr()) if out_image else None, n, C, K, H, W, stride, taps, xe, wexp, oe, 1 if relu else 0,
                 native.stream_ptr(dev)), "dvis_conv_x3_image")
-    return out
+    return out if gn is None else (out, _gn_finalize(part, gn))
 
 
 X3_BNECK = os.environ.get("DVIS_X3_BNECK", "1") != "0"
diff --git a/dvis_plus_amd/native.py b/dvis_plus_amd/native.py
--- a/dvis_plus_amd/native.py
+++ b/dvis_plus_amd/native.py
@@ -63,6 +63,7 @@
     "dvis_bias_relu_maxpool": (_i, [_p, _p, _p, _i64, _i, _i, _i, _p]),
     "dvis_group_norm_affine": (_i, [_p, _p, _p, _p, _p, _i64, _i, _i, _i64, _f, _p]),
     "dvis_scale_shift_act": (_i, [_p, _p, _p, _i64, _i64, _i, _p]),
+    "dvis_group_norm_finalize": (_i, [_p, _p, _p, _p, _p, _i64, _i, _i, _i64, _f, _p]),
     "dvis_upsample_add_affine": (_i, [_p, _p, _p, _p, _p, _i64, _i, _i, _i, _i, _p]),
     "dvis_upsample_add": (_i, [_p, _p, _p, _i64, _i, _i, _i, _i, _p]),
     "dvis_dwconv3x3_tokens": (_i, [_p, _p, _i64, _i, _i, _i, _i, _p, _p, _i, _p]),
@@ -113,6 +114,7 @@
     "dvis_conv1x1_x3_packed_bytes": (_i64, [_i, _i]),
     "dvis_conv1x1_x3_pack": (_i, [_p, _i, _i, _i, _p, _p]),
     "dvis_conv1x1_x3": (_i, [_p, _p, _p, _p, _p, _i, _i, _i, _i, _i, _i, _i, _i, _i, _p]),
+    "dvis_conv_x3_set_extras": (_i, [_p, _p, _p, _i]),
     "dvis_conv1x1_x3_dual": (_i, [_p, _p, _p, _p, _p, _p, _i, _i, _i, _i, _i, _i, _i, _i, _i, _i, _i, _i, _p]),
     "dvis_conv3x3_x3_packed_bytes": (_i64, [_i, _i]),
     "dvis_conv3x3_x3_pack": (_i, [_p, _i, _i, _i, _p, _p]),
diff --git a/dvis_plus_amd/pixel_decoder.py b/dvis_plus_amd/pixel_decoder.py
--- a/dvis_plus_amd/pixel_decoder.py
+++ b/dvis_plus_amd/pixel_decoder.py
@@ -355,13 +355,24 @@
             return Fn.conv3x3_bias_act(x, self.weight, self.bias)
         return F.conv2d(x, self.weight, self.bias, self.stride, self.padding, self.dilation, self.groups)
 
-    def conv_and_affine(self, x):
-        if isinstance(self.norm, nn.GroupNorm) and self.activation is None:
+    def conv_stats(self, x):
+        if isinstance(x, Fn.OperandImage):
+            if Fn.gn_fused_ok(self.norm, self.out_channels, x.H * x.W):
+                return Fn.conv_x3_image(x, self.weight, self.bias, gn=self.norm)
+            y = Fn.conv_x3_image(x, self.weight, self.bias)
+        elif self.kernel_size == (1, 1) and self.stride == (1, 1) and self.groups == 1 and self.padding == (0, 0):
+            return Fn.conv1x1_gn(x, self.weight, self.bias, self.norm)
+        else:
             y = self.conv(x)
-            aff = Fn.group_norm_affine(y, self.norm)
+        return y, Fn.group_norm_affine(y, self.norm)
+
+    def conv_and_affine(self, x, relu_ok=False):
+        if isinstance(self.norm, nn.GroupNorm) and (self.activation is None or (relu_ok and self.activation is F.relu)):
+            y, aff = self.conv_stats(x)
             if aff is not None:
                 return y, aff
-            return self.norm(y), None
+            y = self.norm(y)
+            return (y if self.activation is None else self.activation(y)), None
         return self.forward(x), None
 
     def image_input_ok(self, N, C, H, W, device):
@@ -369,15 +380,21 @@
             and ((self.kernel_size == (3, 3) and self.padding == (1, 1)) or (self.kernel_size == (1, 1) and self.padding == (0, 0))) \
             and C == self.in_channels and Fn.x3_images_ok(N, C, self.out_channels, H, W, device, taps=self.kernel_size[0] ** 2)
 
+    def conv_in_affine(self, x, affine, relu):
+        if self.norm is None and self.activation is None and self.kernel_size == (1, 1) and self.stride == (1, 1) and self.groups == 1 \
+                and self.padding == (0, 0) and Fn.conv1x1_in_affine_ok(x, self.weight):
+            return Fn.conv1x1_in_affine(x, self.weight, self.bias, affine, relu)
+        return self.forward(Fn.scale_shift_act_(x, affine[0], affine[1], relu=relu))
+
     def forward(self, x):
-        if isinstance(x, Fn.OperandImage):
-            x = Fn.conv_x3_image(x, self.weight, self.bias)
-        else:
-            x = self.conv(x)
         if isinstance(self.norm, nn.GroupNorm) and self.activation in (None, F.relu):
-            aff = Fn.group_norm_affine(x, self.norm)
+            x, aff = self.conv_stats(x)
             if aff is not None:
                 return Fn.scale_shift_act_(x, aff[0], aff[1], relu=self.activation is not None)
+        elif isinstance(x, Fn.OperandImage):
+            x = Fn.conv_x3_image(x, self.weight, self.bias)
+        else:
+            x = self.conv(x)
         if self.norm is not None:
             x = self.norm(x)
         if self.activation is not None:
@@ -465,9 +482,11 @@
             for idx, f in enumerate(self.transformer_in_features[::-1]):
                 x = features[f].float().contiguous()
                 conv, gn = self.input_proj[idx][0], self.input_proj[idx][1]
-                s_ = Fn.conv1x1(x, conv.weight, conv.bias) if conv.kernel_size == (1, 1) and conv.stride == (1, 1) \
-                    and conv.padding == (0, 0) and conv.groups == 1 else conv(x)
-                affine = Fn.group_norm_affine(s_, gn)
+                if conv.kernel_size == (1, 1) and conv.stride == (1, 1) and conv.padding == (0, 0) and conv.groups == 1:
+                    s_, affine = Fn.conv1x1_gn(x, conv.weight, conv.bias, gn)
+                else:
+                    s_ = conv(x)
+                    affine = Fn.group_norm_affine(s_, gn)
                 srcs.append(s_ if affine is not None else gn(s_))
                 affines.append(affine)
                 pos.append(self.pe_layer.compute(x.shape[2], x.shape[3], x.device))
@@ -483,17 +502,26 @@
                     out.append(tokens[-1].transpose(1, 2).reshape(bs, -1, h, w))
                 start += h * w
             with Fn.x3_stage("mask_path"):
+                last_affine = None
                 for idx, f in enumerate(self.in_features[:self.num_fpn_levels][::-1]):
                     x = features[f].float().contiguous()
                     cur_fpn, affine = self.lateral_convs[idx].conv_and_affine(x)
                     oc = self.output_convs[idx]
                     if cur_fpn.is_cuda and cur_fpn.dtype == torch.float32 and cur_fpn.is_contiguous() and out[-1].dtype == torch.float32 \
                             and oc.image_input_ok(*cur_fpn.shape, cur_fpn.device):
-                        out.append(oc(Fn.upsample_add_image(cur_fpn, out[-1], affine)))
+                        top = Fn.upsample_add_image(cur_fpn, out[-1], affine)
                     else:
-                        out.append(oc(Fn.upsample_add(cur_fpn, out[-1], affine)))
+                        top = Fn.upsample_add(cur_fpn, out[-1], affine)
+                    if Fn.GN_FUSED and idx + 1 == self.num_fpn_levels and len(out) >= self.maskformer_num_feature_levels \
+                            and top.device.type == "cuda" and not torch.is_grad_enabled():
+                        y, last_affine = oc.conv_and_affine(top, relu_ok=True)
+                        out.append(y)
+                    else:
+                        out.append(oc(top))
                 multi_scale_features = TokenMaps(out[:self.maskformer_num_feature_levels])
                 multi_scale_features.tokens = tokens[:self.maskformer_num_feature_levels]
+                if last_affine is not None:
+                    return self.mask_features.conv_in_affine(out[-1], last_affine, oc.activation is not None), out[0], multi_scale_features
                 return self.mask_features(out[-1]), out[0], multi_scale_features
 
 
diff --git a/include/dvis_hip.h b/include/dvis_hip.h
--- a/include/dvis_hip.h
+++ b/include/dvis_hip.h
@@ -144,6 +144,8 @@
                            int C, int G, int64_t HW, float eps, void *stream);
 int dvis_scale_shift_act(float *x, const float *scale, const float *shift, int64_t planes, int64_t HW, int relu,
                          void *stream);
+int dvis_group_norm_finalize(const double *part, const float *gamma, const float *beta, float *scale, float *shift, int64_t N,
+                             int C, int G, int64_t blocks, float eps, void *stream);
 int dvis_upsample_add_affine(const float *lateral, const float *lat_scale, const float *lat_shift, const float *top,
                              float *out, int64_t planes, int H, int W, int h, int w, void *stream);
 
@@ -234,6 +236,7 @@
 int dvis_conv1x1_x3_pack(const float *w, int K, int C, int wexp, void *packed, void *stream);
 int dvis_conv1x1_x3(const float *x, const void *packed, const float *bias, const float *res, float *y, int N, int C, int K, int H,
                     int W, int stride, int xexp, int wexp, int relu, void *stream);
+int dvis_conv_x3_set_extras(double *gn_part, const float *in_scale, const float *in_shift, int in_relu);
 int dvis_conv1x1_x3_dual(const float *x, const float *x2, const void *packed, const float *bias, const float *res, float *y, int N,
                          int C, int C2, int K, int H, int W, int H2, int W2, int stride2, int xexp, int wexp, int relu, void *stream);
 int64_t dvis_conv3x3_x3_packed_bytes(int C, int K);
```

Result: slower. 401.7 (-2.5%).
